# ziatdinovmax/GPim

Hardware: AMD Instinct MI355X
Metric: GP fit+predict grid-points/sec (higher is better)
Workload: dtype f64; 1 GPU; C2: 256x256 synthetic twisted-lattice image, 25% observed (N=16384, M=65536, d=2), Matern52 exact GP, T=100 Adam its (lr 0.1) + predict; one image per GPU; N=16384, M=65536, kernel=Matern52

## Files before the change

### gpim_amd/_lib.py

```python
import contextlib
import ctypes
import os

import torch

_HERE = os.path.dirname(os.path.abspath(__file__))
LIB_PATH = os.path.join(_HERE, "libgpimhip.so")

OK, E_BADARG, E_HIP, E_NOT_PD, E_NOMEM = 0, -1, -2, -3, -4
KERNEL_IDS = {"RBF": 0, "Matern52": 1, "RationalQuadratic": 2}
ACQ_IDS = {"cb": 0, "ei": 1, "poi": 2}
MAX_DIM, MAX_PARAMS = 4, 8

c_dp = ctypes.c_void_p


class ModelStruct(ctypes.Structure):
    _fields_ = [("kernel", ctypes.c_int32), ("dim", ctypes.c_int32), ("n_ls", ctypes.c_int32),
                ("reserved", ctypes.c_int32), ("amp_lo", ctypes.c_double), ("amp_hi", ctypes.c_double),
                ("ls_lo", ctypes.c_double * MAX_DIM), ("ls_hi", ctypes.c_double * MAX_DIM),
                ("jitter", ctypes.c_double)]


class VgpStruct(ctypes.Structure):
    _fields_ = [("tasks", ctypes.c_int32), ("rank", ctypes.c_int32), ("independent", ctypes.c_int32),
                ("ls_softplus", ctypes.c_int32)]


VGP_MAX_TASKS = 16


class SmStruct(ctypes.Structure):
    _fields_ = [("dim", ctypes.c_int32), ("mixtures", ctypes.c_int32), ("ard", ctypes.c_int32),
                ("reserved", ctypes.c_int32)]


SM_MAX_MIXTURES = 16


class GemmTestStruct(ctypes.Structure):
    _fields_ = [("A", c_dp), ("lda", ctypes.c_int64), ("a_roff", ctypes.c_int32), ("a_coff", ctypes.c_int32),
                ("B", c_dp), ("ldb", ctypes.c_int64), ("b_roff", ctypes.c_int32), ("b_coff", ctypes.c_int32),
                ("C", c_dp), ("ldc", ctypes.c_int64), ("c_roff", ctypes.c_int32), ("c_coff", ctypes.c_int32),
                ("colpart", c_dp), ("ld_colpart", ctypes.c_int64),
                ("alpha", ctypes.c_double), ("beta", ctypes.c_double),
                ("tiles", ctypes.POINTER(ctypes.c_int32)), ("ntiles", ctypes.c_int32),
                ("a_km", ctypes.c_int32), ("b_km", ctypes.c_int32), ("epi", ctypes.c_int32),
                ("krev", ctypes.c_int32), ("chunk", ctypes.c_int32), ("kfix0", ctypes.c_int32), ("kfix1", ctypes.c_int32),
                ("rect_rows", ctypes.c_int32), ("rect_cols", ctypes.c_int32), ("cj_max", ctypes.c_int32),
                ("cmap", ctypes.c_int32), ("rag", ctypes.c_int32), ("inplace", ctypes.c_int32),
                ("bshift", ctypes.c_int32), ("shape_div", ctypes.c_int32),
                ("sA", ctypes.c_int64), ("sB", ctypes.c_int64), ("sC", ctypes.c_int64), ("sColpart", ctypes.c_int64),
                ("batch", ctypes.c_int32)]


GEMM_SHAPES = {"quad": 0, "rowhalf": 1, "8w_lds": 2, "8w": 3, "4w": 4}
EPI_STORE, EPI_COLSUMSQ = 0, 1

_lib = None

_PROTOS = {
    "gpimhip_create": (ctypes.c_int, [ctypes.POINTER(ctypes.c_void_p), ctypes.c_int, ctypes.c_void_p]),
    "gpimhip_destroy": (ctypes.c_int, [ctypes.c_void_p]),
    "gpimhip_last_error": (ctypes.c_char_p, []),
    "gpimhip_version": (ctypes.c_int, []),
    "gpimhip_shutdown": (ctypes.c_int, []),
    "gpimhip_workspace_bytes": (ctypes.c_int64, [ctypes.c_void_p]),
    "gpimhip_sync": (ctypes.c_int, [ctypes.c_void_p]),
    "gpimhip_fit_completed": (ctypes.c_int, [ctypes.c_void_p]),
    "gpimhip_timing_enable": (ctypes.c_int, [ctypes.c_void_p, ctypes.c_int]),
    "gpimhip_timing_read": (ctypes.c_int, [ctypes.c_void_p, ctypes.c_int, ctypes.POINTER(ctypes.c_double),
                                           ctypes.POINTER(ctypes.c_int64)]),
    "gpimhip_kmat": (ctypes.c_int, [ctypes.c_void_p, ctypes.POINTER(ModelStruct), c_dp, ctypes.c_int64, c_dp,
                                    ctypes.c_int64, c_dp, ctypes.c_double, c_dp, ctypes.c_int64]),
    "gpimhip_potrf": (ctypes.c_int, [ctypes.c_void_p, c_dp, ctypes.c_int64, ctypes.c_int64, c_dp]),
    "gpimhip_nll_grad": (ctypes.c_int, [ctypes.c_void_p, ctypes.POINTER(ModelStruct), c_dp, c_dp, ctypes.c_int64,
                                        c_dp, c_dp, c_dp]),
    "gpimhip_fit_exact": (ctypes.c_int, [ctypes.c_void_p, ctypes.POINTER(ModelStruct), c_dp, c_dp, ctypes.c_int64,
                                         c_dp, ctypes.c_double, ctypes.c_int32, c_dp, c_dp]),
    "gpimhip_predict_exact": (ctypes.c_int, [ctypes.c_void_p, ctypes.POINTER(ModelStruct), c_dp, c_dp,
                                             ctypes.c_int64, c_dp, c_dp, ctypes.c_int64, c_dp, c_dp]),
    "gpimhip_sample_exact": (ctypes.c_int, [ctypes.c_void_p, ctypes.POINTER(ModelStruct), c_dp, c_dp, ctypes.c_int64,
                                            c_dp, c_dp, ctypes.c_int64, c_dp, ctypes.c_int32, ctypes.c_int32,
                                            ctypes.c_double, c_dp, c_dp, c_dp]),
    "gpimhip_sample_pathwise": (ctypes.c_int, [ctypes.c_void_p, ctypes.POINTER(ModelStruct), c_dp,
                                               ctypes.POINTER(ctypes.c_int32), ctypes.c_int32,
                                               ctypes.POINTER(ctypes.c_double), c_dp, c_dp, ctypes.c_int64, c_dp, c_dp,
                                               ctypes.c_int32, ctypes.c_int32, ctypes.c_double, c_dp, c_dp]),
    "gpimhip_sample_blocks": (ctypes.c_int, [ctypes.c_void_p, ctypes.POINTER(ModelStruct), c_dp,
                                             ctypes.POINTER(ctypes.c_int32), ctypes.c_int32,
                                             ctypes.POINTER(ctypes.c_double), c_dp, c_dp, c_dp,
                                             ctypes.c_int32, ctypes.c_int32, ctypes.c_double, c_dp, c_dp]),
    "gpimhip_sample_border": (ctypes.c_int, [ctypes.c_void_p, ctypes.POINTER(ModelStruct), c_dp, ctypes.c_int64, c_dp,
                                             ctypes.c_int64, ctypes.c_int32, c_dp, c_dp, ctypes.POINTER(ctypes.c_int32),
                                             ctypes.c_int32, ctypes.POINTER(ctypes.c_double), c_dp, c_dp, ctypes.c_int32,
                                             ctypes.c_int32, ctypes.c_double, c_dp, c_dp]),
    "gpimhip_fit_exact_batched": (ctypes.c_int, [ctypes.c_void_p, ctypes.POINTER(ModelStruct), c_dp, ctypes.c_int64,
                                                 c_dp, ctypes.c_int64, ctypes.c_int32, c_dp, ctypes.c_double,
                                                 ctypes.c_int32, c_dp, c_dp]),
    "gpimhip_predict_exact_batched": (ctypes.c_int, [ctypes.c_void_p, ctypes.POINTER(ModelStruct), c_dp,
                                                     ctypes.c_int64, c_dp, ctypes.c_int64, ctypes.c_int32, c_dp,
                                                     c_dp, ctypes.c_int64, c_dp, c_dp]),
    "gpimhip_vfe_nll_grad": (ctypes.c_int, [ctypes.c_void_p, ctypes.POINTER(ModelStruct), c_dp, c_dp, ctypes.c_int64,
                                            ctypes.c_int64, c_dp, c_dp, c_dp]),
    "gpimhip_fit_vfe": (ctypes.c_int, [ctypes.c_void_p, ctypes.POINTER(ModelStruct), c_dp, c_dp, ctypes.c_int64,
                                       ctypes.c_int64, c_dp, ctypes.c_double, ctypes.c_int32, c_dp, c_dp, c_dp]),
    "gpimhip_predict_vfe": (ctypes.c_int, [ctypes.c_void_p, ctypes.POINTER(ModelStruct), c_dp, c_dp, ctypes.c_int64,
                                           ctypes.c_int64, c_dp, c_dp, ctypes.c_int64, c_dp, c_dp]),
    "gpimhip_fit_vfe_batched": (ctypes.c_int, [ctypes.c_void_p, ctypes.POINTER(ModelStruct), c_dp, ctypes.c_int64, c_dp,
                                               ctypes.c_int64, ctypes.c_int64, ctypes.c_int32, c_dp, ctypes.c_double,
                                               ctypes.c_int32, c_dp, c_dp, c_dp]),
    "gpimhip_predict_vfe_batched": (ctypes.c_int, [ctypes.c_void_p, ctypes.POINTER(ModelStruct), c_dp, ctypes.c_int64, c_dp,
                                                   ctypes.c_int64, ctypes.c_int64, ctypes.c_int32, c_dp, c_dp,
                                                   ctypes.c_int64, ctypes.c_int64, c_dp, c_dp]),
    "gpimhip_kron_nll_grad": (ctypes.c_int, [ctypes.c_void_p, ctypes.POINTER(ModelStruct), ctypes.c_int32,
                                             ctypes.POINTER(ctypes.c_int32), c_dp, c_dp, c_dp, c_dp, c_dp]),
    "gpimhip_fit_kron": (ctypes.c_int, [ctypes.c_void_p, ctypes.POINTER(ModelStruct), ctypes.c_int32,
                                        ctypes.POINTER(ctypes.c_int32), c_dp, c_dp, c_dp, ctypes.c_double,
                                        ctypes.c_int32, c_dp, c_dp]),
    "gpimhip_predict_kron": (ctypes.c_int, [ctypes.c_void_p, ctypes.POINTER(ModelStruct), ctypes.c_int32,
                                            ctypes.POINTER(ctypes.c_int32), c_dp, c_dp, c_dp,
                                            ctypes.POINTER(ctypes.c_int32), c_dp, c_dp, c_dp]),
    "gpimhip_pkron_nll_grad": (ctypes.c_int, [ctypes.c_void_p, ctypes.POINTER(ModelStruct), c_dp, ctypes.c_int64, ctypes.c_int32,
                                              ctypes.c_int32, ctypes.POINTER(ctypes.c_int32), ctypes.POINTER(ctypes.c_int32),
                                              c_dp, c_dp, c_dp, c_dp, c_dp]),
    "gpimhip_fit_pkron": (ctypes.c_int, [ctypes.c_void_p, ctypes.POINTER(ModelStruct), c_dp, ctypes.c_int64, ctypes.c_int32,
                                         ctypes.c_int32, ctypes.POINTER(ctypes.c_int32), ctypes.POINTER(ctypes.c_int32),
                                         c_dp, c_dp, c_dp, ctypes.c_double, ctypes.c_int32, c_dp, c_dp]),
    "gpimhip_predict_pkron": (ctypes.c_int, [ctypes.c_void_p, ctypes.POINTER(ModelStruct), c_dp, ctypes.c_int64, ctypes.c_int32,
                                             ctypes.c_int32, ctypes.POINTER(ctypes.c_int32), ctypes.POINTER(ctypes.c_int32),
                                             c_dp, c_dp, c_dp, c_dp, ctypes.c_int64, ctypes.POINTER(ctypes.c_int32), c_dp,
                                             c_dp, c_dp]),
    "gpimhip_sample_pkron": (ctypes.c_int, [ctypes.c_void_p, ctypes.POINTER(ModelStruct), c_dp, ctypes.c_int64, ctypes.c_int32,
                                            ctypes.c_int32, ctypes.POINTER(ctypes.c_int32), ctypes.POINTER(ctypes.c_int32),
                                            c_dp, c_dp, c_dp, c_dp, ctypes.c_int64, ctypes.POINTER(ctypes.c_int32), c_dp,
                                            c_dp, ctypes.c_int64, ctypes.POINTER(ctypes.c_int32), ctypes.POINTER(ctypes.c_int32),
                                            ctypes.POINTER(ctypes.c_int32), c_dp, ctypes.POINTER(ctypes.c_int32),
                                            ctypes.POINTER(ctypes.c_int32), c_dp, ctypes.c_int32, ctypes.c_int32,
                                            ctypes.c_double, c_dp, c_dp]),
    "gpimhip_sample_kron": (ctypes.c_int, [ctypes.c_void_p, ctypes.POINTER(ModelStruct), ctypes.c_int32,
                                           ctypes.POINTER(ctypes.c_int32), c_dp, c_dp, c_dp,
                                           ctypes.POINTER(ctypes.c_int32), c_dp,
                                           ctypes.POINTER(ctypes.c_int32), c_dp,
                                           ctypes.POINTER(ctypes.c_int32), ctypes.POINTER(ctypes.c_int32),
                                           c_dp, ctypes.c_int32, ctypes.c_int32, ctypes.c_double, c_dp, c_dp]),
    "gpimhip_acq": (ctypes.c_int, [ctypes.c_void_p, ctypes.c_int32, c_dp, c_dp, ctypes.c_int64, ctypes.c_double,
                                   ctypes.c_double, c_dp, c_dp]),
    "gpimhip_nanmax": (ctypes.c_int, [ctypes.c_void_p, c_dp, ctypes.c_int64, c_dp]),
    "gpimhip_topk": (ctypes.c_int, [ctypes.c_void_p, c_dp, ctypes.c_int64, ctypes.c_int32, ctypes.c_int32,
                                    c_dp, c_dp, c_dp]),
    "gpimhip_dist_begin": (ctypes.c_int, [ctypes.c_void_p, ctypes.c_int64]),
    "gpimhip_dist_panel_factor": (ctypes.c_int, [ctypes.c_void_p, c_dp, ctypes.c_int64, ctypes.c_int32,
                                                 ctypes.c_int32, c_dp, c_dp]),
    "gpimhip_dist_setup": (ctypes.c_int, [ctypes.c_void_p, ctypes.c_int64, ctypes.c_int32, ctypes.c_int32]),
    "gpimhip_dist_panel_pack": (ctypes.c_int, [ctypes.c_void_p, c_dp, ctypes.c_int64, ctypes.c_int32, ctypes.c_int32,
                                               c_dp, ctypes.c_int64]),
    "gpimhip_dist_update": (ctypes.c_int, [ctypes.c_void_p, c_dp, ctypes.c_int64, ctypes.c_int32, c_dp, ctypes.c_int64,
                                           ctypes.c_int32, ctypes.c_int32]),
    "gpimhip_dist_solve_update": (ctypes.c_int, [ctypes.c_void_p, c_dp, ctypes.c_int64, ctypes.c_int32, c_dp,
                                                 ctypes.c_int64, ctypes.c_int64, c_dp, ctypes.c_int64, c_dp,
                                                 ctypes.c_int32]),
    "gpimhip_dist_solve_update2": (ctypes.c_int, [ctypes.c_void_p, c_dp, ctypes.c_int64, ctypes.c_int32, c_dp,
                                                  ctypes.c_int64, ctypes.c_int64, c_dp, ctypes.c_int64, c_dp,
                                                  ctypes.c_int32, ctypes.c_int32]),
    "gpimhip_dist_kmat_cols": (ctypes.c_int, [ctypes.c_void_p, ctypes.POINTER(ModelStruct), c_dp, ctypes.c_int64, c_dp,
                                              ctypes.c_int64, ctypes.c_int64, c_dp, ctypes.c_int64]),
    "gpimhip_dist_kinv_update": (ctypes.c_int, [ctypes.c_void_p, c_dp, ctypes.c_int64, ctypes.c_int32, c_dp,
                                                ctypes.c_int64, c_dp, ctypes.c_int64]),
    "gpimhip_dist_kinv_update_n": (ctypes.c_int, [ctypes.c_void_p, c_dp, ctypes.c_int64, ctypes.c_int32, ctypes.c_int32, c_dp,
                                                  ctypes.c_int64, c_dp, ctypes.c_int64]),
    "gpimhip_dist_grad_sums": (ctypes.c_int, [ctypes.c_void_p, ctypes.POINTER(ModelStruct), c_dp, ctypes.c_int64, c_dp,
                                              c_dp, ctypes.c_int64, c_dp, c_dp]),
    "gpimhip_dist_finalize": (ctypes.c_int, [ctypes.c_void_p, ctypes.POINTER(ModelStruct), ctypes.c_int64, c_dp, c_dp,
                                             ctypes.c_double, ctypes.c_double, ctypes.c_double, ctypes.c_int32, c_dp,
                                             c_dp, c_dp]),
    "gpimhip_dist_finalize_dev": (ctypes.c_int, [ctypes.c_void_p, ctypes.POINTER(ModelStruct), ctypes.c_int64, c_dp, c_dp,
                                                 c_dp, ctypes.c_double, ctypes.c_int32, c_dp, c_dp, c_dp]),
    "gpimhip_set_precision": (ctypes.c_int, [ctypes.c_void_p, ctypes.c_int32]),
    "gpimhip_set_reflection_shard": (ctypes.c_int, [ctypes.c_void_p, ctypes.c_int32, ctypes.c_int32, ctypes.c_int32, ctypes.c_int32]),
    "gpimhip_refl_sums": (ctypes.c_int, [ctypes.c_void_p, ctypes.POINTER(ModelStruct), c_dp, c_dp, ctypes.c_int64, ctypes.c_int32,
                                         c_dp, c_dp]),
    "gpimhip_set_reflection": (ctypes.c_int, [ctypes.c_void_p, ctypes.c_int32, ctypes.POINTER(ctypes.c_double), c_dp,
                                              ctypes.c_int64, ctypes.c_int64]),
    "gpimhip_set_border": (ctypes.c_int, [ctypes.c_void_p, ctypes.c_int32, ctypes.c_void_p, c_dp]),
    "gpimhip_nll_grad_batched": (ctypes.c_int, [ctypes.c_void_p, ctypes.POINTER(ModelStruct), c_dp, ctypes.c_int64, c_dp,
                                                ctypes.c_int64, ctypes.c_int32, c_dp, c_dp, c_dp]),
    "gpimhip_acquire_exact": (ctypes.c_int, [ctypes.c_void_p, ctypes.POINTER(ModelStruct), c_dp, c_dp, ctypes.c_int64,
                                             c_dp, c_dp, ctypes.c_int64, c_dp, ctypes.c_int64, ctypes.c_int32,
                                             ctypes.c_double, ctypes.c_double, c_dp, c_dp, c_dp, c_dp]),
    "gpimhip_thin_batch": (ctypes.c_int, [ctypes.c_void_p, c_dp, c_dp, ctypes.c_int32, ctypes.c_int32, c_dp,
                                          ctypes.c_double, ctypes.c_int32, c_dp, c_dp]),
    "gpimhip_dist_vec_forward": (ctypes.c_int, [ctypes.c_void_p, c_dp, ctypes.c_int64, ctypes.c_int32, ctypes.c_int32,
                                                c_dp, c_dp, c_dp, c_dp]),
    "gpimhip_dist_vec_backward": (ctypes.c_int, [ctypes.c_void_p, c_dp, ctypes.c_int64, ctypes.c_int32, ctypes.c_int32,
                                                 c_dp, c_dp, c_dp, c_dp]),
    "gpimhip_matvec_t": (ctypes.c_int, [ctypes.c_void_p, c_dp, ctypes.c_int64, ctypes.c_int64, ctypes.c_int64, c_dp,
                                        c_dp]),
    "gpimhip_step_plan_host": (ctypes.c_int, [ctypes.c_int32, ctypes.c_int32, ctypes.POINTER(ctypes.c_int32),
                                              ctypes.c_int64, ctypes.POINTER(ctypes.c_int64)]),
    "gpimhip_step_plan_host_f32": (ctypes.c_int, [ctypes.c_int32, ctypes.c_int32, ctypes.POINTER(ctypes.c_int32),
                                                  ctypes.c_int64, ctypes.POINTER(ctypes.c_int64),
                                                  ctypes.POINTER(ctypes.c_int32)]),
    "gpimhip_gemm_tiles": (ctypes.c_int, [ctypes.c_void_p, ctypes.POINTER(GemmTestStruct)]),
    "gpimhip_gemm_shape_host": (ctypes.c_int, [ctypes.c_int32, ctypes.c_int32, ctypes.c_int32, ctypes.c_int32,
                                               ctypes.c_int64, ctypes.c_int64, ctypes.c_int32, ctypes.c_int32]),
    "gpimhip_gemm_tile_pos_host": (ctypes.c_int, [ctypes.c_int32, ctypes.c_int32, ctypes.c_int32, ctypes.c_int32,
                                                  ctypes.c_int32, ctypes.c_int32, ctypes.POINTER(ctypes.c_int32),
                                                  ctypes.POINTER(ctypes.c_int32)]),
    "gpimhip_gemm_rect_tile_host": (ctypes.c_int, [ctypes.c_int32, ctypes.c_int32, ctypes.c_int32, ctypes.c_int32,
                                                   ctypes.POINTER(ctypes.c_int32), ctypes.POINTER(ctypes.c_int32)]),
    "gpimhip_kron_eigh": (ctypes.c_int, [ctypes.c_void_p, ctypes.c_int32, ctypes.POINTER(ctypes.c_int32), c_dp,
                                         ctypes.POINTER(ctypes.c_double), ctypes.c_int32, c_dp, c_dp,
                                         ctypes.POINTER(ctypes.c_int32), ctypes.POINTER(ctypes.c_int32),
                                         ctypes.POINTER(ctypes.c_double), ctypes.POINTER(ctypes.c_int32)]),
    "gpimhip_vgp_nll_grad": (ctypes.c_int, [ctypes.c_void_p, ctypes.POINTER(ModelStruct), ctypes.POINTER(VgpStruct), c_dp,
                                            c_dp, ctypes.c_int64, c_dp, c_dp, c_dp]),
    "gpimhip_fit_vgp": (ctypes.c_int, [ctypes.c_void_p, ctypes.POINTER(ModelStruct), ctypes.POINTER(VgpStruct), c_dp, c_dp,
                                       ctypes.c_int64, c_dp, ctypes.c_double, ctypes.c_int32, c_dp, c_dp]),
    "gpimhip_predict_vgp": (ctypes.c_int, [ctypes.c_void_p, ctypes.POINTER(ModelStruct), ctypes.POINTER(VgpStruct), c_dp,
                                           c_dp, ctypes.c_int64, c_dp, c_dp, ctypes.c_int64, c_dp, c_dp]),
    "gpimhip_sample_vgp": (ctypes.c_int, [ctypes.c_void_p, ctypes.POINTER(ModelStruct), ctypes.POINTER(VgpStruct), c_dp, c_dp,
                                          ctypes.c_int64, c_dp, c_dp, ctypes.c_int64, c_dp, ctypes.c_int32, ctypes.c_int32,
                                          ctypes.c_double, c_dp, c_dp, c_dp]),
    "gpimhip_sample_vgp_blocks": (ctypes.c_int, [ctypes.c_void_p, ctypes.POINTER(ModelStruct), ctypes.POINTER(VgpStruct), c_dp,
                                                 ctypes.POINTER(ctypes.c_int32), ctypes.c_int32,
                                                 ctypes.POINTER(ctypes.c_double), c_dp, c_dp, c_dp, ctypes.c_int32,
                                                 ctypes.c_int32, ctypes.c_double, c_dp, c_dp]),
    "gpimhip_sm_kmat": (ctypes.c_int, [ctypes.c_void_p, ctypes.POINTER(SmStruct), c_dp, ctypes.c_int64, c_dp, ctypes.c_int64,
                                       c_dp, c_dp, ctypes.c_int64]),
    "gpimhip_sm_nll_grad": (ctypes.c_int, [ctypes.c_void_p, ctypes.POINTER(SmStruct), c_dp, c_dp, ctypes.c_int64, c_dp, c_dp,
                                           c_dp]),
    "gpimhip_fit_sm": (ctypes.c_int, [ctypes.c_void_p, ctypes.POINTER(SmStruct), c_dp, c_dp, ctypes.c_int64, c_dp,
                                      ctypes.c_double, ctypes.c_int32, c_dp, c_dp]),
    "gpimhip_predict_sm": (ctypes.c_int, [ctypes.c_void_p, ctypes.POINTER(SmStruct), c_dp, c_dp, ctypes.c_int64, c_dp, c_dp,
                                          ctypes.c_int64, c_dp, c_dp]),
    "gpimhip_sample_sm": (ctypes.c_int, [ctypes.c_void_p, ctypes.POINTER(SmStruct), c_dp, c_dp, ctypes.c_int64, c_dp, c_dp,
                                         ctypes.c_int64, c_dp, ctypes.c_int32, ctypes.c_int32, ctypes.c_double, c_dp, c_dp,
                                         c_dp]),
    "gpimhip_sample_sm_pathwise": (ctypes.c_int, [ctypes.c_void_p, ctypes.POINTER(SmStruct), c_dp,
                                                  ctypes.POINTER(ctypes.c_int32), ctypes.c_int32,
                                                  ctypes.POINTER(ctypes.c_double), c_dp, c_dp, ctypes.c_int64, c_dp, c_dp,
                                                  ctypes.c_int32, ctypes.c_int32, ctypes.c_double, c_dp, c_dp]),
    "gpimhip_sample_sm_blocks": (ctypes.c_int, [ctypes.c_void_p, ctypes.POINTER(SmStruct), c_dp,
                                                ctypes.POINTER(ctypes.c_int32), ctypes.c_int32,
                                                ctypes.POINTER(ctypes.c_double), c_dp, c_dp, c_dp,
                                                ctypes.c_int32, ctypes.c_int32, ctypes.c_double, c_dp, c_dp]),
    "gpimhip_sm_nll_grad_batched": (ctypes.c_int, [ctypes.c_void_p, ctypes.POINTER(SmStruct), c_dp, c_dp, c_dp, ctypes.c_int64,
                                                   ctypes.c_int32, c_dp, c_dp, c_dp]),
    "gpimhip_fit_sm_batched": (ctypes.c_int, [ctypes.c_void_p, ctypes.POINTER(SmStruct), c_dp, c_dp, c_dp, ctypes.c_int64,
                                              ctypes.c_int32, c_dp, ctypes.c_double, ctypes.c_int32, c_dp, c_dp]),
    "gpimhip_predict_sm_batched": (ctypes.c_int, [ctypes.c_void_p, ctypes.POINTER(SmStruct), c_dp, c_dp, c_dp, ctypes.c_int64,
                                                  ctypes.c_int32, c_dp, c_dp, ctypes.c_int64, c_dp, c_dp]),
}
EXPORTS = tuple(_PROTOS)


def load():
    global _lib
    if _lib is not None:
        return _lib
    if not os.path.exists(LIB_PATH):
        raise RuntimeError(
            "gpim_amd: %s is missing -- build it with `python -m gpim_amd._build` "
            "(hipcc --offload-arch=gfx950). There is no CPU fallback." % LIB_PATH)
    try:
        lib = ctypes.CDLL(LIB_PATH)
    except OSError as e:
        raise RuntimeError("gpim_amd: cannot load %s: %s. There is no CPU fallback." % (LIB_PATH, e))
    for name, (res, args) in _PROTOS.items():
        fn = getattr(lib, name)
        fn.restype, fn.argtypes = res, args
    _lib = lib
    import atexit
    atexit.register(_shutdown)
    return lib


import weakref

_live = weakref.WeakSet()


def _shutdown():
    import gc
    gc.collect()
    for h in list(_live):
        try:
            h.close()
        except Exception:
            pass
    try:
        if torch.cuda.is_available() and torch.cuda.is_initialized():
            torch.cuda.synchronize()
            _lib.gpimhip_shutdown()
    except Exception:
        pass


def require_gpu():
    if not torch.cuda.is_available():
        raise RuntimeError("gpim_amd: no HIP device visible to torch; the MI355X engine has no CPU fallback")
    return torch.device("cuda", torch.cuda.current_device())


class NotPositiveDefiniteError(torch.linalg.LinAlgError if hasattr(torch.linalg, "LinAlgError") else RuntimeError):
    """Raised where torch.linalg.cholesky would raise in the reference (gpr.py:192,248)."""


def check(rc):
    if rc == OK:
        return
    msg = load().gpimhip_last_error().decode()
    if rc == E_NOT_PD:
        raise NotPositiveDefiniteError("linalg.cholesky: " + msg)
    if rc == E_BADARG:
        raise ValueError("gpimhip: bad argument. " + msg)
    if rc == E_NOMEM:
        raise MemoryError("gpimhip: " + msg)
    raise RuntimeError("gpimhip: HIP error. " + msg)


class Handle:

    def __init__(self, precision="double", stream=None):
        self.device = require_gpu()
        lib = load()
        h = ctypes.c_void_p()
        stream = (stream or torch.cuda.current_stream(self.device)).cuda_stream
        check(lib.gpimhip_create(ctypes.byref(h), self.device.index, ctypes.c_void_p(stream)))
        self._h = h
        self.lib = lib
        _live.add(self)
        self.precision = precision
        if precision == "single":
            check(lib.gpimhip_set_precision(h, 32))

    @property
    def h(self):
        return self._h

    def close(self):
        if getattr(self, "_h", None):
            self.lib.gpimhip_destroy(self._h)
            self._h = None

    def __del__(self):
        try:
            self.close()
        except Exception:
            pass


def ptr(t):
    if t is None:
        return None
    assert t.is_cuda and (t.is_contiguous() or (t.dim() == 2 and t.stride(1) == 1))
    return ctypes.c_void_p(t.data_ptr())


@contextlib.contextmanager
def reflection(handle, blocks, var_count=0, border=None, shard=None):
    lib, h = handle.lib, handle.h
    mode = lambda *args: check(lib.gpimhip_set_reflection(h, *args))
    mode(blocks.mask, blocks.twoc, ptr(blocks.wts), blocks.n_total, int(var_count))
    try:
        if border is not None:
            M, q_d, coef_d = border
            check(lib.gpimhip_set_border(h, M, None if q_d is None else ctypes.c_void_p(q_d.data_ptr()), ptr(coef_d)))
        if shard is not None:
            check(lib.gpimhip_set_reflection_shard(h, *(int(v) for v in shard)))
        yield
    finally:
        mode(0, None, None, 0, 0)
```

### gpim_amd/csrc/api.hip

```cpp
#include <math.h>
#include <stdio.h>
#include <string.h>
#include <stdlib.h>
#include <algorithm>
#include <chrono>
#include <atomic>
#include <mutex>
#include "common.hpp"
#include "border.hpp"
#include "vgp.hpp"
#include "pkron.hpp"
#include "sm.hpp"
#include "sample.hpp"

static thread_local std::string g_err;
void gpim_set_error(const std::string& s) { g_err = s; }

int deal_chunk(int ntiles) { return std::max(1, std::min(64, ntiles / 512)); }
#define EAGER_MIN_PANELS 12


static inline int64_t mat_doubles(const gpimhip_ctx* h, int64_t elements) { return h->fp32 ? (elements + 1) / 2 : elements; }

static void ws_release_matrix(gpimhip_ctx* h) {
    dev_release(h, h->A, h->B, h->Tm, h->dinv, h->dinvB, h->pcopy, h->ypad, h->z, h->alpha, h->logdet_part, h->grad_part,
                h->gemv_part, h->fin_counter, h->theta, h->adam_m, h->adam_v, h->iter);
    h->np = 0;
    h->ws_batch = 0;
}

int ws_ensure_b(gpimhip_ctx* h, int64_t N, int B, int padded, bool matrices) {
    const int64_t np = pad_to(std::max<int64_t>(N, 1), NB);
    const int64_t ld = np + ((padded && np >= 1024) ? (h->fp32 ? 32 : 16) : 0);
    if (np == h->np && B == h->ws_batch && ld == h->ld && (h->A != nullptr || !matrices)) return GPIMHIP_OK;
    HIP_TRY(hipStreamSynchronize(h->stream));
    ws_release_matrix(h);
    const int64_t nb = np / NB;
    h->np = np;
    h->ws_batch = B;
    h->ld = ld;
    int rc = GPIMHIP_OK;
    if ((matrices && ((rc = h->A.alloc(h, mat_doubles(h, B * np * ld))) ||
                      (rc = h->B.alloc(h, mat_doubles(h, B * np * ld))) ||
                      (rc = h->Tm.alloc(h, mat_doubles(h, B * np * ld))))) ||
        (rc = h->dinv.alloc(h, mat_doubles(h, B * nb * NB * NB))) ||
        (rc = h->dinvB.alloc(h, B * nb * NB * NB)) ||
        (rc = h->pcopy.alloc(h, (int64_t)B * NB * NB)) ||
        (rc = h->ypad.alloc(h, B * np)) || (rc = h->z.alloc(h, B * np)) ||
        (rc = h->alpha.alloc(h, B * np)) || (rc = h->logdet_part.alloc(h, B * nb)) ||
        (rc = h->grad_part.alloc(h, B * nb * (nb + 1) / 2 * 8)) || (rc = h->gemv_part.alloc(h, B * (int64_t)gemv_tri_chunks(np) * np)) || (rc = h->fin_counter.alloc(h, (int64_t)B)) || (rc = h->theta.alloc(h, (int64_t)B)) ||
        (rc = h->adam_m.alloc(h, (int64_t)B * MAXP)) || (rc = h->adam_v.alloc(h, (int64_t)B * MAXP)) ||
        (rc = h->iter.alloc(h, (int64_t)B))) {
        ws_release_matrix(h);
        return rc;
    }
    HIP_TRY(hipMemsetAsync(h->fin_counter, 0, (size_t)B * sizeof(uint32_t), h->stream));
    if (matrices) {
        HIP_TRY(hipMemsetAsync(h->Tm, 0, (size_t)mat_doubles(h, B * np * ld) * sizeof(double), h->stream));
        HIP_TRY(hipMemsetAsync(h->B, 0, (size_t)mat_doubles(h, B * np * ld) * sizeof(double), h->stream));
    }
    if (h->fp32 && h->refine.cap < 10 * (int64_t)B * np) {
        h->refine.release(h);
        if ((rc = h->refine.alloc(h, 10 * (int64_t)B * np))) {
            ws_release_matrix(h);
            return rc;
        }
    }
    if (matrices) {
        rc = plan_ensure(h, (int)nb);
        if (rc == GPIMHIP_OK) rc = h->fp32 ? step_plan_ensure(h, (int)nb) : step_plan_ensure_inv(h, (int)nb);
        if (rc != GPIMHIP_OK) { ws_release_matrix(h); return rc; }
    }
    return GPIMHIP_OK;
}
int ws_ensure(gpimhip_ctx* h, int64_t N) { return ws_ensure_b(h, N, h->nbatch, 0); }
static int ws_ensure_padded(gpimhip_ctx* h, int64_t N) { return ws_ensure_b(h, N, h->nbatch, 1); }

static void ws_release_predict(gpimhip_ctx* h) {
    dev_release(h, h->Ks, h->colpart, h->mean_tmp);
    for (auto& pl : h->pred_lists) pl.tiles.release(h);
    h->pred_lists.clear();
    h->pred_tiles = nullptr;
    h->pred_ntiles = 0;
    h->ks_rows = h->ks_cols = 0;
    h->ks_batch = 0;
}

int ws_ensure_predict(gpimhip_ctx* h, int64_t np, int64_t mc) {
    const int B = h->nbatch;
    if (!(h->ks_rows == np && h->ks_batch == B && mc <= h->ks_cols)) {
        HIP_TRY(hipStreamSynchronize(h->stream));
        const int64_t cap = (h->ks_rows == np && h->ks_batch == B) ? std::max(mc, h->ks_cols) : mc;
        ws_release_predict(h);
        h->ks_rows = np;
        h->ks_cols = cap;
        h->ks_batch = B;
        int rc = GPIMHIP_OK;
        if ((rc = h->Ks.alloc(h, mat_doubles(h, B * np * (cap + 16)))) || (rc = h->colpart.alloc(h, B * (np / NB) * cap)) ||
            (rc = h->mean_tmp.alloc(h, B * cap))) {
            ws_release_predict(h);
            return rc;
        }
    }
    const int nb = (int)(np / NB), nc = (int)(mc / NB);
    for (auto& pl : h->pred_lists)
        if (pl.nc == nc) {
            h->pred_tiles = pl.tiles;
            h->pred_ntiles = pl.tiles.cap;
            return GPIMHIP_OK;
        }
    std::vector<TileDesc> tl;
    tl.reserve((size_t)nb * nc);
    for (int ig = (nb - 1) / 8; ig >= 0; --ig)
        for (int jg = 0; jg <= (nc - 1) / 8; ++jg)
            for (int ci = std::min(nb - 1, ig * 8 + 7); ci >= ig * 8; --ci)
                for (int cj = jg * 8; cj < std::min(nc, jg * 8 + 8); ++cj) tl.push_back({ci, cj, 0, ci + 1});
    gpimhip_ctx::PredList pl{nc, {}};
    GP_TRY(pl.tiles.alloc(h, (int64_t)tl.size()));
    HIP_TRY(hipMemcpyAsync(pl.tiles, tl.data(), tl.size() * sizeof(TileDesc), hipMemcpyHostToDevice, h->stream));
    HIP_TRY(hipStreamSynchronize(h->stream));
    h->pred_lists.push_back(pl);
    h->pred_tiles = pl.tiles;
    h->pred_ntiles = pl.tiles.cap;
    return GPIMHIP_OK;
}

static void lower_patch_order(std::vector<TileDesc>& out, int lo, int hi, int kb0, int kb1) {
    for (int ig = lo / 8; ig <= (hi - 1) / 8; ++ig)
        for (int jg = lo / 8; jg <= ig; ++jg)
            for (int i = std::max(lo, ig * 8); i < std::min(hi, ig * 8 + 8); ++i)
                for (int j = std::max(lo, jg * 8); j < std::min(hi, jg * 8 + 8); ++j)
                    if (j <= i) out.push_back({i, j, kb0, kb1});
}

template <typename F>
static void rect_patch_order(std::vector<TileDesc>& out, int r0, int r1, int c0, int c1, bool rows_desc,
                             bool col_major, F krange) {
    const int nrg = (r1 - r0 + 7) / 8, ncg = (c1 - c0 + 7) / 8;
    const int nouter = col_major ? ncg : nrg, ninner = col_major ? nrg : ncg;
    for (int a = 0; a < nouter; ++a)
        for (int bq = 0; bq < ninner; ++bq) {
            int ig = col_major ? bq : a, jg = col_major ? a : bq;
            if (rows_desc) ig = nrg - 1 - ig;
            for (int i = r0 + ig * 8; i < std::min(r1, r0 + ig * 8 + 8); ++i)
                for (int j = c0 + jg * 8; j < std::min(c1, c0 + jg * 8 + 8); ++j) {
                    int k0, k1;
                    krange(i, j, k0, k1);
                    out.push_back({i, j, k0, k1});
                }
        }
}

struct TriNode { int lo, mid, hi; };
static int tri_build(int lo, int hi, std::vector<std::vector<TriNode>>& levels) {
    if (hi - lo <= 1) return 0;
    const int mid = lo + (hi - lo + 1) / 2;
    const int hl = tri_build(lo, mid, levels), hr = tri_build(mid, hi, levels);
    const int ht = 1 + std::max(hl, hr);
    if ((int)levels.size() < ht) levels.resize(ht);
    levels[ht - 1].push_back({lo, mid, hi});
    return ht;
}

int plan_ensure(gpimhip_ctx* h, int nb) {
    LinalgPlan& P = h->plan;
    if (P.nb == nb) return GPIMHIP_OK;
    if (P.d_tiles) { (void)hipFree(P.d_tiles); P.d_tiles = nullptr; }
    std::vector<TileDesc> tl;
    auto mark = [&](size_t start) { return PlanRange{(int64_t)start, (int32_t)(tl.size() - start)}; };
    std::vector<std::vector<TriNode>> levels;
    tri_build(0, nb, levels);
    P.tri_t.clear();
    P.tri_x.clear();
    auto sort_longest_first = [&](size_t nnodes, size_t start) {
        if (nnodes < 2 || tl.size() - start <= 512) return;
        std::stable_sort(tl.begin() + start, tl.end(),
                         [](const TileDesc& a, const TileDesc& b) { return a.kb1 - a.kb0 > b.kb1 - b.kb0; });
    };
    for (auto& lv : levels) {
        size_t s = tl.size();
        for (auto& nd : lv)
            rect_patch_order(tl, nd.mid, nd.hi, nd.lo, nd.mid, false, true,
                             [&](int, int cj, int& k0, int& k1) { k0 = cj; k1 = nd.mid; });
        sort_longest_first(lv.size(), s);
        P.tri_t.push_back(mark(s));
        s = tl.size();
        for (auto& nd : lv)
            rect_patch_order(tl, nd.mid, nd.hi, nd.lo, nd.mid, true, false,
                             [&](int ci, int, int& k0, int& k1) { k0 = nd.mid; k1 = ci + 1; });
        sort_longest_first(lv.size(), s);
        P.tri_x.push_back(mark(s));
    }
    {
        size_t s = tl.size();
        const int PR = 2, PC = 32;
        for (int ig = 0; ig <= (nb - 1) / PR; ++ig)
            for (int jg = 0; jg * PC <= std::min(nb - 1, ig * PR + PR - 1); ++jg)
                for (int i = ig * PR; i < std::min(nb, ig * PR + PR); ++i)
                    for (int j = jg * PC; j < std::min(nb, jg * PC + PC); ++j)
                        if (j <= i) tl.push_back({i, j, i, nb});
        P.lauum = mark(s);
    }
    P.n_tiles = (int64_t)tl.size();
    void* q = nullptr;
    HIP_TRY(hipMalloc(&q, std::max<size_t>(tl.size(), 1) * sizeof(TileDesc)));
    P.d_tiles = (TileDesc*)q;
    HIP_TRY(hipMemcpyAsync(P.d_tiles, tl.data(), tl.size() * sizeof(TileDesc), hipMemcpyHostToDevice, h->stream));
    HIP_TRY(hipStreamSynchronize(h->stream));
    P.nb = nb;
    return GPIMHIP_OK;
}

GemmArgs gemm_args(const double* A, int64_t lda, const double* B, int64_t ldb, double* C, int64_t ldc,
                   double alpha, double beta, const TileDesc* tiles, int n, int64_t rows) {
    GemmArgs g;
    memset(&g, 0, sizeof(g));
    g.A = A; g.lda = lda; g.B = B; g.ldb = ldb; g.C = C; g.ldc = ldc;
    g.alpha = alpha; g.beta = beta; g.tiles = tiles; g.ntiles = n;
    g.sA = rows * lda; g.sB = rows * ldb; g.sC = rows * ldc;
    return g;
}

struct SideStreams {
    hipStream_t capture = nullptr;
    bool capture_tried = false;
};
static std::mutex g_side_mutex;
static SideStreams g_side[64];
static std::atomic<int> g_side_generation{0};
static void side_refresh(gpimhip_ctx* h) {
    const int g = g_side_generation.load();
    if (h->side_generation == g) return;
    h->side_generation = g;
    h->capture_stream = nullptr;
    h->capture_stream_tried = false;
}
static std::mutex g_capture_mutex[64];
static void capture_lock(gpimhip_ctx* h) { g_capture_mutex[h->device & 63].lock(); }
static void capture_unlock(gpimhip_ctx* h) { g_capture_mutex[h->device & 63].unlock(); }

static hipStream_t ensure_capture_stream(gpimhip_ctx* h) {
    side_refresh(h);
    if (!h->capture_stream && !h->capture_stream_tried) {
        h->capture_stream_tried = true;
        std::lock_guard<std::mutex> lock(g_side_mutex);
        SideStreams& S = g_side[h->device & 63];
        if (!S.capture_tried) {
            S.capture_tried = true;
            if (hipStreamCreateWithFlags(&S.capture, hipStreamNonBlocking) != hipSuccess) S.capture = nullptr;
        }
        h->capture_stream = S.capture;
    }
    return h->capture_stream;
}

int launch_potrf(gpimhip_ctx* h, double* A, int64_t np, int64_t ld, int32_t* info) {
    return launch_potrf_steps(h, A, np, ld, info, nullptr);
}

int launch_trtri(gpimhip_ctx* h, double* A, double* Tm, int64_t np, int64_t ld) {
    const int nb = (int)(np / NB);
    GP_TRY(plan_ensure(h, nb));
    const LinalgPlan& P = h->plan;
    GP_TRY(launch_diag_inv_copy(h, A, ld, nb));
    for (size_t lv = 0; lv < P.tri_t.size(); ++lv) {
        GemmArgs g1 = gemm_args(A, ld, A, ld, Tm, ld, 1.0, 0.0, P.d_tiles + P.tri_t[lv].off, P.tri_t[lv].n, h->np);
        g1.chunk = deal_chunk(g1.ntiles);
        g1.krev = 1;
        GP_TRY(launch_gemm(h, false, true, EPI_STORE, g1));
        GemmArgs g2 = gemm_args(A, ld, Tm, ld, A, ld, -1.0, 0.0, P.d_tiles + P.tri_x[lv].off, P.tri_x[lv].n, h->np);
        g2.chunk = deal_chunk(g2.ntiles);
        GP_TRY(launch_gemm(h, false, true, EPI_STORE, g2));
    }
    return GPIMHIP_OK;
}

int launch_potrf_inv(gpimhip_ctx* h, double* A, double* Tm, int64_t np, int64_t ld, int32_t* info, int rag) {
    if (!h->fp32) return launch_potrf_steps(h, A, np, ld, info, Tm, rag);
    { StageTimer t(h, 0); GP_TRY(launch_potrf_steps(h, A, np, ld, info, nullptr)); }
    StageTimer t(h, 1);
    return launch_trtri(h, A, Tm, np, ld);
}

int launch_lauum(gpimhip_ctx* h, const double* A, double* B, int64_t np, int64_t ld, int rag) {
    const int nb = (int)(np / NB);
    GP_TRY(plan_ensure(h, nb));
    const LinalgPlan& P = h->plan;
    GemmArgs g = gemm_args(A, ld, A, ld, B, ld, 1.0, 0.0, P.d_tiles + P.lauum.off, P.lauum.n, h->np);
    g.chunk = deal_chunk(g.ntiles);
    g.krev = 1;
    g.rag = h->fp32 ? 0 : rag;
    return launch_gemm(h, true, true, EPI_STORE, g);
}

BorderWs* bws(const gpimhip_ctx* h) { return (BorderWs*)h->border; }
bool border_on(const gpimhip_ctx* h) { return h->refl.mask && h->border && bws(h)->M > 0; }

static void border_free_bufs(gpimhip_ctx* h, BorderWs* w) {
    dev_release(h, w->C, w->Y, w->tv, w->scal, w->uo, w->tiles_y, w->tiles_upd, w->R, w->rsq);
    w->np = 0; w->B = 0; w->n_y = w->n_upd = 0; w->r_cols = 0;
}
static void border_release(gpimhip_ctx* h) {
    BorderWs* w = bws(h);
    if (!w) return;
    border_free_bufs(h, w);
    if (w->sub) gpimhip_destroy(w->sub);
    delete w;
    h->border = nullptr;
}

static int border_ensure(gpimhip_ctx* h, int T = 1) {
    BorderWs* w = bws(h);
    const int64_t mp = pad_to(w->M, NB);
    if (!w->sub) GP_TRY(gpimhip_create(&w->sub, h->device, h->stream));
    w->sub->nbatch = T;
    w->sub->stream = h->stream;
    GP_TRY(ws_ensure_b(w->sub, w->M, T, 1));
    if (w->np == h->np && w->B == h->nbatch && w->T == T && w->mp == mp && w->C) return GPIMHIP_OK;
    HIP_TRY(hipStreamSynchronize(h->stream));
    border_free_bufs(h, w);
    w->mp = mp; w->np = h->np; w->B = h->nbatch; w->T = T;
    const int nb = (int)(h->np / NB), nm = (int)(mp / NB);
    std::vector<TileDesc> ty, tu;
    for (int ci = 0; ci < nb; ++ci)
        for (int cj = 0; cj < nm; ++cj) ty.push_back({ci, cj, 0, cj + 1});
    lower_patch_order(tu, 0, nb, 0, nm);
    w->n_y = (int)ty.size();
    w->n_upd = (int)tu.size();
    int rc = GPIMHIP_OK;
    if ((rc = w->C.alloc(h, (int64_t)w->B * w->np * mp)) || (rc = w->Y.alloc(h, (int64_t)w->B * w->np * mp)) ||
        (rc = w->tv.alloc(h, 2 * mp * T)) || (rc = w->scal.alloc(h, 2 * T)) || (rc = w->tiles_y.alloc(h, w->n_y)) ||
        (rc = w->tiles_upd.alloc(h, w->n_upd))) {
        border_free_bufs(h, w);
        return rc;
    }
    HIP_TRY(hipMemcpyAsync(w->tiles_y, ty.data(), ty.size() * sizeof(TileDesc), hipMemcpyHostToDevice, h->stream));
    HIP_TRY(hipMemcpyAsync(w->tiles_upd, tu.data(), tu.size() * sizeof(TileDesc), hipMemcpyHostToDevice, h->stream));
    HIP_TRY(hipStreamSynchronize(h->stream));
    return GPIMHIP_OK;
}
static int border_ensure_r(gpimhip_ctx* h, int64_t cols) {
    BorderWs* w = bws(h);
    if (w->r_cols >= cols && w->R) return GPIMHIP_OK;
    HIP_TRY(hipStreamSynchronize(h->stream));
    dev_release(h, w->R, w->rsq);
    w->r_cols = 0;
    int rc = GPIMHIP_OK;
    if ((rc = w->R.alloc(h, w->mp * cols * w->T)) || (rc = w->rsq.alloc(h, cols * w->T))) {
        w->R.release(h);
        return rc;
    }
    w->r_cols = cols;
    return GPIMHIP_OK;
}

static int border_iter(gpimhip_ctx* h, int64_t nq, bool update_inverse) {
    BorderWs* w = bws(h);
    gpimhip_ctx* sub = w->sub;
    sub->stream = h->stream;
    const int64_t mp = w->mp;
    GP_TRY(launch_border_gather_s(h, w, h->B, h->ld, sub->A, sub->ld));
    GP_TRY(launch_potrf_inv(sub, sub->A, sub->Tm, mp, sub->ld, sub->info, 0));
    GP_TRY(launch_border_tidy(h, w, sub->A, sub->ld));
    GP_TRY(launch_border_gather_c(h, w, h->B, h->ld, nq));
    {
        GemmArgs g = gemm_args(w->C, mp, sub->A, sub->ld, w->Y, mp, 1.0, 0.0, w->tiles_y, w->n_y, h->np);
        g.sB = sub->np * sub->ld;
        g.bshift = __builtin_ctz((unsigned)(h->nbatch / w->T));
        g.chunk = deal_chunk(g.ntiles);
        GP_TRY(launch_gemm(h, false, false, EPI_STORE, g));
    }
    GP_TRY(launch_border_vectors(h, w, sub->A, sub->ld, sub->logdet_part, (int)(mp / NB), h->alpha));
    if (update_inverse) {
// ... 1789 lines not shown
```

### gpim_amd/csrc/cholstep.hip

```cpp
#include <stdlib.h>
#include <string.h>
#include <algorithm>
#include <functional>
#include "potf2_body.hpp"
#include "gemm_body.hpp"

#ifndef STEP_W
#define STEP_W 4
#endif

#define TILE_COPY (1 << 19)

struct StepArgs {
    double* A; int64_t ld; int kblk; int nb;
    double* dinv_all; double* dinvB_all; double* logdet; int32_t* info;
    int col_off;
    int potf2;
    int pb_off, pb_cnt, hb_off, hb_cnt, swap;
    double* Tm;
    double* Pcopy;
    GemmArgs g;
};

template <int FTM, int FTN, bool ALONE, bool RAG = false>
__global__ __launch_bounds__(NTH, ALONE ? 2 : 4) void chol_step_kernel(StepArgs a) {
    constexpr int SM0 = POTF2_SMEM_DOUBLES > gemm_smem_doubles<FTM, FTN, 2>() ? POTF2_SMEM_DOUBLES : gemm_smem_doubles<FTM, FTN, 2>();
    static_assert(SM0 * 8 <= 80 * 1024, "two workgroups per CU");
    constexpr int SM = ALONE ? 84 * 128 : SM0;
    __shared__ __attribute__((aligned(16))) double smem[SM];
    const int b = a.swap ? blockIdx.y : blockIdx.x;
    const int by = a.swap ? blockIdx.x : blockIdx.y;
    if (b >= 8) {
        if (by >= a.hb_cnt) return;
        const int pb = by + a.hb_off;
        int quad;
        const int pos = gemm_tile_pos<FTM, FTN>(a.g.ntiles, a.g.chunk, b - 8, quad);
        TileDesc t = a.g.tiles[pos];
        const int kind = (t.kb1 >> 16) & 7;
        const bool copy = (t.kb1 & TILE_COPY) != 0;
        t.kb1 &= 0xffff;
        if (kind == 0) {
            if (copy && a.Pcopy) {
                GemmArgs g = a.g;
                g.C2 = a.Pcopy + (int64_t)pb * (NB * NB);
                gemm_tile_core<false, false, EPI_STORE, 8, FTM, FTN, 2, RAG>(g, t, quad, pb, smem);
            } else {
                gemm_tile_core<false, false, EPI_STORE, 8, FTM, FTN, 2, RAG>(a.g, t, quad, pb, smem);
            }
        } else {
            GemmArgs g = a.g;
            if (kind <= 2) { g.C = a.Tm; g.alpha = 1.0; g.beta = kind == 2 ? 1.0 : 0.0; }
            else { g.B = a.Tm; g.alpha = -1.0; g.beta = kind == 4 ? 1.0 : 0.0; }
            gemm_tile_core<false, true, EPI_STORE, 8, FTM, FTN, 2, RAG>(g, t, quad, pb, smem);
        }
        return;
    }
    if (b != 0 || !a.potf2 || by >= a.pb_cnt) return;
    if (!ALONE) __builtin_amdgcn_s_setprio(3);
    potf2_body<double, ALONE && FI_LOOKAHEAD>(smem, by + a.pb_off, a.A, a.ld, a.kblk, a.dinv_all, a.dinvB_all, a.logdet, a.info, a.nb,
                                              a.col_off, a.Tm != nullptr);
}

template <int WPE>
__global__ __launch_bounds__(256, WPE) void panel_solve_kernel(double* __restrict__ A, int64_t ld, int kblk, int nb,
                                                            const double* __restrict__ dinvB_all, int b_off) {
    constexpr int LDS_LD = 130;
    constexpr int ROWS = 32, MTS = ROWS / 16;
    __shared__ __attribute__((aligned(16))) double S[ROWS * LDS_LD];
    const int tid = threadIdx.x, lane = tid & 63, wave = tid >> 6;
    const int by = blockIdx.y + b_off;
    A += (int64_t)by * nb * NB * ld;
    const d2* DB = reinterpret_cast<const d2*>(dinvB_all + ((int64_t)by * nb + kblk) * (NB * NB));
    double* P = A + ((int64_t)(kblk + 1) * NB + (int64_t)blockIdx.x * ROWS) * ld + (int64_t)kblk * NB;
#pragma unroll
    for (int i = 0; i < ROWS / 4; ++i) {
        const int row = wave * (ROWS / 4) + i;
        __builtin_amdgcn_global_load_lds((const __attribute__((address_space(1))) void*)(P + (int64_t)row * ld + lane * 2),
                                         (__attribute__((address_space(3))) void*)(S + row * LDS_LD), 16, 0, 0);
    }
    const int t0 = wave, t1 = 7 - wave, n0 = 2 * t0 + 2;
    d2 bf[18];
#pragma unroll
    for (int q = 0; q < 18; ++q) {
        const int t = q < n0 ? t0 : t1, s2 = q < n0 ? q : q - n0;
        bf[q] = DB[(t * 16 + s2) * 64 + lane];
    }
    asm volatile("s_waitcnt vmcnt(0)" ::: "memory");
    __syncthreads();
    const d4 zero = (d4){0.0, 0.0, 0.0, 0.0};
    d4 acc[2][MTS];
#pragma unroll
    for (int x = 0; x < 2; ++x)
#pragma unroll
        for (int mt = 0; mt < MTS; ++mt) acc[x][mt] = zero;
    const double* Sa = S + (lane & 15) * LDS_LD + (lane >> 4);
#pragma unroll
    for (int q = 0; q < 18; ++q) {
        const bool first = q < n0;
        const int s2 = first ? q : q - n0;
#pragma unroll
        for (int e = 0; e < 2; ++e) {
            const int s = 2 * s2 + e;
#pragma unroll
            for (int mt = 0; mt < MTS; ++mt) {
                const double av = Sa[mt * 16 * LDS_LD + 4 * s];
                if (first) acc[0][mt] = __builtin_amdgcn_mfma_f64_16x16x4f64(av, bf[q][e], acc[0][mt], 0, 0, 0);
                else acc[1][mt] = __builtin_amdgcn_mfma_f64_16x16x4f64(av, bf[q][e], acc[1][mt], 0, 0, 0);
            }
        }
    }
#pragma unroll
    for (int x = 0; x < 2; ++x) {
        const int t = x == 0 ? t0 : t1;
#pragma unroll
        for (int mt = 0; mt < MTS; ++mt)
#pragma unroll
            for (int rg = 0; rg < 4; ++rg)
                P[(int64_t)(mt * 16 + (lane >> 4) + 4 * rg) * ld + t * 16 + (lane & 15)] = acc[x][mt][rg];
    }
}

__global__ __launch_bounds__(256, 2) void diag_update_kernel(double* __restrict__ A, int64_t ld, int kblk, int nb, int b_off) {
    constexpr int LDS_LD = 130;
    __shared__ __attribute__((aligned(16))) double S[64 * LDS_LD];
    const int tid = threadIdx.x, lane = tid & 63, wave = tid >> 6;
    A += (int64_t)(blockIdx.y + b_off) * nb * NB * ld;
    const int jj = kblk + 1 + blockIdx.x / 10, q = blockIdx.x % 10;
    const int a = q < 1 ? 0 : q < 3 ? 1 : q < 6 ? 2 : 3, b = q - a * (a + 1) / 2;
    const double* Pa = A + ((int64_t)jj * NB + a * 32) * ld + (int64_t)kblk * NB;
    const double* Pb = A + ((int64_t)jj * NB + b * 32) * ld + (int64_t)kblk * NB;
#pragma unroll
    for (int i = 0; i < 8; ++i) {
        const int row = wave * 8 + i;
        __builtin_amdgcn_global_load_lds((const __attribute__((address_space(1))) void*)(Pa + (int64_t)row * ld + lane * 2),
                                         (__attribute__((address_space(3))) void*)(S + row * LDS_LD), 16, 0, 0);
        __builtin_amdgcn_global_load_lds((const __attribute__((address_space(1))) void*)(Pb + (int64_t)row * ld + lane * 2),
                                         (__attribute__((address_space(3))) void*)(S + (32 + row) * LDS_LD), 16, 0, 0);
    }
    const int wm = wave >> 1, wn = wave & 1;
    double* C = A + ((int64_t)jj * NB + a * 32 + wm * 16 + (lane >> 4)) * ld + (int64_t)jj * NB + b * 32 + wn * 16 + (lane & 15);
    double cv[4];
#pragma unroll
    for (int rg = 0; rg < 4; ++rg) cv[rg] = C[(int64_t)(4 * rg) * ld];
    asm volatile("s_waitcnt vmcnt(0)" ::: "memory");
    __syncthreads();
    d4 acc0 = (d4){0.0, 0.0, 0.0, 0.0}, acc1 = acc0;
    const double* Sa = S + (wm * 16 + (lane & 15)) * LDS_LD + (lane >> 4);
    const double* Sb = S + (32 + wn * 16 + (lane & 15)) * LDS_LD + (lane >> 4);
#pragma unroll
    for (int s = 0; s < 32; s += 2) {
        acc0 = __builtin_amdgcn_mfma_f64_16x16x4f64(Sa[4 * s], Sb[4 * s], acc0, 0, 0, 0);
        acc1 = __builtin_amdgcn_mfma_f64_16x16x4f64(Sa[4 * s + 4], Sb[4 * s + 4], acc1, 0, 0, 0);
    }
#pragma unroll
    for (int rg = 0; rg < 4; ++rg) C[(int64_t)(4 * rg) * ld] = cv[rg] - (acc0[rg] + acc1[rg]);
}

template <int ROWS>
__global__ __launch_bounds__(512, 2) void panel_solve_diag_kernel(double* __restrict__ A, int64_t ld, int kblk, int nb,
                                                                  const double* __restrict__ dinvB_all,
                                                                  const double* __restrict__ Pcopy, int b_off) {
    constexpr int LDS_LD = 130, MTS = ROWS / 16, NS = NB / ROWS, NDIAG = NS * (NS + 1) / 2;
    __shared__ __attribute__((aligned(16))) double S[2 * ROWS * LDS_LD];
    const int tid = threadIdx.x, lane = tid & 63, wave = (tid >> 6) & 3, half = tid >> 8;
    const int by = blockIdx.y + b_off;
    A += (int64_t)by * nb * NB * ld;
    Pcopy += (int64_t)by * (NB * NB);
    const d2* DB = reinterpret_cast<const d2*>(dinvB_all + ((int64_t)by * nb + kblk) * (NB * NB));
    const bool diag = blockIdx.x < NDIAG;
    int a = 0, b = 0;
    if (diag) {
        const int q = blockIdx.x;
        while ((a + 1) * (a + 2) / 2 <= q) ++a;
        b = q - a * (a + 1) / 2;
    }
    const int jj = kblk + 1;
    const int strip = diag ? (half == 0 ? a : b) : NS + 2 * (int)(blockIdx.x - NDIAG) + half;
    const bool work = !diag || half == 0 || b != a;
    double* P = A + ((int64_t)jj * NB + strip * ROWS) * ld + (int64_t)kblk * NB;
    double* Ss = S + half * ROWS * LDS_LD;
    if (work) {
#pragma unroll
        for (int i = 0; i < ROWS / 4; ++i) {
            const int row = wave * (ROWS / 4) + i;
            const double* src = diag ? Pcopy + (strip * ROWS + row) * NB + lane * 2 : P + (int64_t)row * ld + lane * 2;
            __builtin_amdgcn_global_load_lds((const __attribute__((address_space(1))) void*)src,
                                             (__attribute__((address_space(3))) void*)(Ss + row * LDS_LD), 16, 0, 0);
        }
    }
    const int t0 = wave, t1 = 7 - wave, n0 = 2 * t0 + 2;
    d2 bf[18];
    if (work) {
#pragma unroll
        for (int q = 0; q < 18; ++q) {
            const int t = q < n0 ? t0 : t1, s2 = q < n0 ? q : q - n0;
            bf[q] = DB[(t * 16 + s2) * 64 + lane];
        }
    }
    const int wt = tid >> 6, wm = wt / MTS, wn = wt % MTS;
    const bool syrk = diag && wt < MTS * MTS;
    double* C = A + ((int64_t)jj * NB + a * ROWS + wm * 16 + (lane >> 4)) * ld + (int64_t)jj * NB + b * ROWS + wn * 16 + (lane & 15);
    double cv[4] = {0.0, 0.0, 0.0, 0.0};
    if (syrk) {
#pragma unroll
        for (int rg = 0; rg < 4; ++rg) cv[rg] = C[(int64_t)(4 * rg) * ld];
    }
    asm volatile("s_waitcnt vmcnt(0)" ::: "memory");
    __syncthreads();
    const d4 zero = (d4){0.0, 0.0, 0.0, 0.0};
    d4 acc[2][MTS];
#pragma unroll
    for (int x = 0; x < 2; ++x)
#pragma unroll
        for (int mt = 0; mt < MTS; ++mt) acc[x][mt] = zero;
    if (work) {
        const double* Sa = Ss + (lane & 15) * LDS_LD + (lane >> 4);
#pragma unroll
        for (int q = 0; q < 18; ++q) {
            const bool first = q < n0;
            const int s2 = first ? q : q - n0;
#pragma unroll
            for (int e = 0; e < 2; ++e) {
                const int s = 2 * s2 + e;
#pragma unroll
                for (int mt = 0; mt < MTS; ++mt) {
                    const double av = Sa[mt * 16 * LDS_LD + 4 * s];
                    if (first) acc[0][mt] = __builtin_amdgcn_mfma_f64_16x16x4f64(av, bf[q][e], acc[0][mt], 0, 0, 0);
                    else acc[1][mt] = __builtin_amdgcn_mfma_f64_16x16x4f64(av, bf[q][e], acc[1][mt], 0, 0, 0);
                }
            }
        }
        if (!diag || (a == b && half == 0)) {
#pragma unroll
            for (int x = 0; x < 2; ++x) {
                const int t = x == 0 ? t0 : t1;
#pragma unroll
                for (int mt = 0; mt < MTS; ++mt)
#pragma unroll
                    for (int rg = 0; rg < 4; ++rg)
                        P[(int64_t)(mt * 16 + (lane >> 4) + 4 * rg) * ld + t * 16 + (lane & 15)] = acc[x][mt][rg];
            }
        }
    }
    if (!diag) return;
    __syncthreads();
    if (work) {
#pragma unroll
        for (int x = 0; x < 2; ++x) {
            const int t = x == 0 ? t0 : t1;
#pragma unroll
            for (int mt = 0; mt < MTS; ++mt)
#pragma unroll
                for (int rg = 0; rg < 4; ++rg)
                    Ss[(mt * 16 + (lane >> 4) + 4 * rg) * LDS_LD + t * 16 + (lane & 15)] = acc[x][mt][rg];
        }
    }
    __syncthreads();
    if (!syrk) return;
    d4 acc0 = zero, acc1 = zero;
    const double* Sa = S + (wm * 16 + (lane & 15)) * LDS_LD + (lane >> 4);
    const double* Sb = S + ((b != a ? ROWS : 0) + wn * 16 + (lane & 15)) * LDS_LD + (lane >> 4);
#pragma unroll
    for (int s = 0; s < 32; s += 2) {
        acc0 = __builtin_amdgcn_mfma_f64_16x16x4f64(Sa[4 * s], Sb[4 * s], acc0, 0, 0, 0);
        acc1 = __builtin_amdgcn_mfma_f64_16x16x4f64(Sa[4 * s + 4], Sb[4 * s + 4], acc1, 0, 0, 0);
    }
#pragma unroll
    for (int rg = 0; rg < 4; ++rg) C[(int64_t)(4 * rg) * ld] = cv[rg] - (acc0[rg] + acc1[rg]);
}

static void lower_patches(std::vector<TileDesc>& out, int lo, int hi, int kb0, int kb1) {
    for (int ig = lo / 8; ig <= (hi - 1) / 8; ++ig)
        for (int jg = lo / 8; jg <= ig; ++jg)
            for (int i = std::max(lo, ig * 8); i < std::min(hi, ig * 8 + 8); ++i)
                for (int j = std::max(lo, jg * 8); j < std::min(hi, jg * 8 + 8); ++j)
                    if (j <= i) out.push_back({i, j, kb0, kb1});
}

static bool pair_mode32(int nb) { return nb >= 160; }
static int fill_cap32(int nb) { return pair_mode32(nb) ? 64 : (nb < 88 ? (1 << 30) : 128); }

struct HostSim {
    std::vector<double> slot;
    double makespan = 0.0;
    explicit HostSim(int S) : slot(S, 0.0) {}
    static double cost(const TileDesc& t) { return ((t.kb1 & 0xffff) - t.kb0) + 0.5; }
    double peek() const { return slot.front(); }
    void add(double c) {
        std::pop_heap(slot.begin(), slot.end(), std::greater<double>());
        slot.back() += c;
        makespan = std::max(makespan, slot.back());
        std::push_heap(slot.begin(), slot.end(), std::greater<double>());
    }
    bool try_add(double c, int q, double limit) {
        double t[4];
        for (int w = 0; w < q; ++w) {
            std::pop_heap(slot.begin(), slot.end() - w, std::greater<double>());
            t[w] = slot[slot.size() - 1 - w];
        }
        const bool ok = t[q - 1] + c <= limit;
        for (int w = q - 1; w >= 0; --w) {
            if (ok) { slot[slot.size() - 1 - w] = t[w] + c; makespan = std::max(makespan, t[w] + c); }
            std::push_heap(slot.begin(), slot.end() - w, std::greater<double>());
        }
        return ok;
    }
};
#define HOST_SLOTS 512
static double wg_cost(int depth, int q) { return q == 4 ? 0.14 * depth + 0.24 : (q == 2 ? 0.34 * depth + 0.3 : depth + 0.5); }

static void plan_updates(int nb, std::vector<std::vector<TileDesc>>& fill) {
#ifndef STEP_W_CHAIN
#define STEP_W_CHAIN 3
#endif
#ifndef STEP_W_CHAIN_MIN
#define STEP_W_CHAIN_MIN 16
#endif
    const int W = (nb >= STEP_W_CHAIN_MIN && nb < 64) ? STEP_W_CHAIN : STEP_W, S = HOST_SLOTS;
    const int npanel = (nb + W - 1) / W;
    auto by_depth = [](const TileDesc& a, const TileDesc& b) { return (a.kb1 - a.kb0) > (b.kb1 - b.kb0); };
    auto col_update = [&](std::vector<TileDesc>& tl, int p0, int j) {
        const int kb0 = std::max(0, p0 - W);
        if (j > kb0)
            for (int i = j + 1; i < nb; ++i) tl.push_back({i, j, kb0, j});
        if (j + 1 < nb) {
            const int kd = std::max(0, ((j + 1) / W) * W - W);
            if (j > kd) tl.push_back({j + 1, j + 1, kd, j});
        }
    };
    if (nb < 64) {
        for (int p = 0; p < npanel; ++p) {
            const int p0 = p * W, p1 = std::min(p0 + W, nb), ncol = p1 - p0;
            std::vector<TileDesc> bulk;
            if (p > 0 && p0 + W < nb) lower_patches(bulk, p0 + W, nb, p0 - W, p0);
            const size_t per = (bulk.size() + ncol - 1) / ncol;
            size_t taken = 0;
            for (int j = p0; j < p1; ++j) {
                col_update(fill[j], p0, j);
                for (size_t q = 0; q < per && taken < bulk.size(); ++q) fill[j].push_back(bulk[taken++]);
            }
        }
        return;
    }
    std::vector<int> pend((size_t)nb * nb, 0);
    for (int p = 0; p < npanel; ++p) {
        const int p0 = p * W, p1 = std::min(p0 + W, nb);
        const int rem = nb - p0 - W;
        std::vector<TileDesc> req, opt;
        if (p > 0 && rem > 0) {
            const int c0 = p0 + W, c1 = std::min(p0 + 2 * W, nb);
            for (int i = c0; i < nb; ++i)
                for (int jj = c0; jj < std::min(c1, i + 1); ++jj) req.push_back({i, jj, pend[(size_t)i * nb + jj], p0});
            if (c1 < nb) lower_patches(opt, c1, nb, 0, p0);
            for (auto& t : opt) t.kb0 = pend[(size_t)t.ci * nb + t.cj];
        }
        const bool bulk_regime = rem >= 64;
#ifndef PLAN_FLUSH
#define PLAN_FLUSH 2
#endif
        constexpr int F = PLAN_FLUSH;
        auto due = [&](const TileDesc& t) { return (t.kb1 - t.kb0) >= F * W || (((t.ci >> 3) + (t.cj >> 3)) % F) == (p % F); };
        double due_cost = 0.0;
        size_t n_due = 0;
        if (bulk_regime) {
            std::stable_sort(opt.begin(), opt.end(), [&](const TileDesc& a, const TileDesc& b) {
                const int da = due(a), db = due(b);
                if (da != db) return da > db;
                return da ? by_depth(a, b) : false;
            });
            for (auto& t : opt)
                if (due(t)) { ++n_due; due_cost += HostSim::cost(t); }
        }
        size_t rtaken = 0, otaken = 0;
        for (int j = p0; j < p1; ++j) {
            const int left = p1 - j;
            std::vector<TileDesc>& tl = fill[j];
            col_update(tl, p0, j);
            const size_t nreq = (req.size() - rtaken + left - 1) / left;
            for (size_t q = 0; q < nreq; ++q) tl.push_back(req[rtaken++]);
            if (!bulk_regime) {
                const size_t nopt = (opt.size() - otaken + left - 1) / left;
                for (size_t q = 0; q < nopt; ++q) tl.push_back(opt[otaken++]);
            } else {
                HostSim sim(S);
                sim.add(1.0);
                std::stable_sort(tl.begin(), tl.end(), by_depth);
                double base = 0.0;
                for (auto& t : tl) { sim.add(HostSim::cost(t)); base += HostSim::cost(t); }
                const double per_slot = (base + due_cost / left) / S;
                const double unit = F * W + 0.5;
                const double target = std::max(sim.makespan, unit * std::max(1.0, std::floor(per_slot / unit + 0.5)));
                double got = 0.0;
                while (otaken < opt.size() && sim.peek() + HostSim::cost(opt[otaken]) <= target + 0.25) {
                    const double c = HostSim::cost(opt[otaken]);
                    sim.add(c);
                    if (otaken < n_due) got += c;
                    tl.push_back(opt[otaken++]);
                }
                due_cost -= std::min(due_cost, got);
            }
            std::stable_sort(tl.begin(), tl.end(), by_depth);
            for (auto& t : tl)
                if (t.cj >= p0 + W) pend[(size_t)t.ci * nb + t.cj] = t.kb1;
        }
    }
}

enum { TK_UPDATE = 0, TK_T_FIRST = 1, TK_T_ACC = 2, TK_X_FIRST = 3, TK_X_ACC = 4 };
struct TriOp { int ci, cj, k0, k1, kp; };
struct TriNodeS {
    int lo, mid, hi, left, right, height;
    int t_done = 1 << 30, x_done = 1 << 30;
    std::vector<TriOp> T, X;
    size_t t_open = 0, x_open = 0;
};
static int tri_nodes(int lo, int hi, std::vector<TriNodeS>& nodes) {
    TriNodeS n;
    n.lo = lo; n.hi = hi; n.mid = lo; n.left = n.right = -1; n.height = 0;
    if (hi - lo <= 1) {
        n.t_done = n.x_done = lo;
        nodes.push_back(n);
        return (int)nodes.size() - 1;
    }
    n.mid = lo + (hi - lo + 1) / 2;
    n.left = tri_nodes(lo, n.mid, nodes);
    n.right = tri_nodes(n.mid, hi, nodes);
    n.height = 1 + std::max(nodes[n.left].height, nodes[n.right].height);
    for (int cj = lo; cj < n.mid; ++cj)
        for (int ci = n.mid; ci < hi; ++ci) n.T.push_back({ci, cj, cj, n.mid, cj});
    for (int ci = hi - 1; ci >= n.mid; --ci)
        for (int cj = lo; cj < n.mid; ++cj) n.X.push_back({ci, cj, n.mid, ci + 1, n.mid});
    n.t_open = n.T.size();
    n.x_open = n.X.size();
    nodes.push_back(n);
    return (int)nodes.size() - 1;
}

#ifndef BATCH_QUAD_MAX
#define BATCH_QUAD_MAX 700
#endif
static int host_shape(int64_t update_kblocks, int quad_max = 2000) { return update_kblocks <= quad_max ? 4 : (update_kblocks <= 2800 ? 2 : 1); }

#ifndef PAIR_MIN_QUADS
#define PAIR_MIN_QUADS 300
#endif
#ifndef PAIR_MIN_DEPTH10
#define PAIR_MIN_DEPTH10 30
#endif
static bool pair_rule(size_t ntiles, int64_t kblocks) { return 4 * ntiles >= PAIR_MIN_QUADS && 10 * kblocks >= PAIR_MIN_DEPTH10 * (int64_t)ntiles; }
static bool plan_inverse(int nb, std::vector<std::vector<TileDesc>>& fill, std::vector<std::vector<TileDesc>>& post,
                         std::vector<uint8_t>& pair) {
    std::vector<TriNodeS> nodes;
    tri_nodes(0, nb, nodes);
    std::vector<int> order(nodes.size());
    for (size_t i = 0; i < order.size(); ++i) order[i] = (int)i;
    std::stable_sort(order.begin(), order.end(), [&](int a, int b) { return nodes[a].height < nodes[b].height; });
    size_t open_nodes = 0;
    for (auto& n : nodes) open_nodes += (n.height > 0);
#ifndef PLAN_CHAIN
#define PLAN_CHAIN 0.8
#endif
    const double CHAIN = PLAN_CHAIN;
    for (int L = 0; open_nodes > 0; ++L) {
        const bool hosted = L < nb;
        if (!hosted) post.emplace_back();
        std::vector<TileDesc>& out = hosted ? fill[L] : post.back();
        int64_t upd = 0;
        for (auto& t : out) upd += t.kb1 - t.kb0;
        const int q = hosted ? host_shape(upd) : 1;
        const int cd = !hosted ? (1 << 20) : 6;
        const bool two = hosted && q == 4 && pair_rule(out.size(), upd);
        if (hosted) pair[L] = two;
#ifndef PLAN_PAIR_SLOW
#define PLAN_PAIR_SLOW 1.7
#endif
#ifndef PLAN_PAIR_CHAIN
#define PLAN_PAIR_CHAIN 0.3
#endif
        const double slow = two ? PLAN_PAIR_SLOW : 1.0, chain = two ? CHAIN + PLAN_PAIR_CHAIN : CHAIN;
        HostSim sim(q == 1 || two ? HOST_SLOTS : HOST_SLOTS / 2);
        double target = 1e30;
        if (hosted) {
            sim.add(chain);
            for (auto& t : out)
                for (int w = 0; w < q; ++w) sim.add(slow * wg_cost(t.kb1 - t.kb0, q));
            target = std::max(sim.makespan, chain);
        }
        bool full = false;
        for (int idx : order) {
            TriNodeS& n = nodes[idx];
            if (n.height == 0 || n.x_open == 0 || full) continue;
            const bool t_phase = n.t_open > 0;
            if (t_phase ? !(nodes[n.left].x_done < L && n.mid <= L) : !(n.t_done < L && nodes[n.right].x_done < L && n.hi <= L)) continue;
            std::vector<TriOp>& ops = t_phase ? n.T : n.X;
            size_t& open = t_phase ? n.t_open : n.x_open;
            for (auto& o : ops) {
                if (o.kp >= o.k1) continue;
                int depth = std::min(o.k1 - o.kp, cd);
                if (hosted) {
                    while (depth >= 1 && !sim.try_add(slow * wg_cost(depth, q), q, target + 0.02)) --depth;
                    if (depth < 1) { full = true; break; }
                } else {
                    for (int w = 0; w < q; ++w) sim.add(wg_cost(depth, q));
                }
                const int k1 = o.kp + depth;
                const int kind = t_phase ? (o.kp == o.k0 ? TK_T_FIRST : TK_T_ACC) : (o.kp == o.k0 ? TK_X_FIRST : TK_X_ACC);
                out.push_back({o.ci, o.cj, o.kp, k1 | (kind << 16)});
                o.kp = k1;
                if (o.kp >= o.k1 && --open == 0) {
                    if (t_phase) n.t_done = L;
                    else { n.x_done = L; --open_nodes; }
                }
            }
        }
        std::stable_sort(out.begin(), out.end(), [](const TileDesc& a, const TileDesc& b) {
            return ((a.kb1 & 0xffff) - a.kb0) > ((b.kb1 & 0xffff) - b.kb0);
        });
        if (!hosted && out.empty()) post.pop_back();
        if (L > nb + 4 * 64) return false;
    }
    return true;
}

static void plan_updates_f32(int nb, std::vector<std::vector<TileDesc>>& fill, std::vector<std::vector<TileDesc>>& rest,
                             std::vector<int>& ndiag) {
    const int W = STEP_W;
    const int npanel = (nb + W - 1) / W;
    fill.assign(nb, {});
    rest.assign(npanel, {});
    ndiag.assign(nb, 0);
    for (int p = 0; p < npanel; ++p) {
        const int p0 = p * W, p1 = std::min(p0 + W, nb), ncol = p1 - p0;
        std::vector<TileDesc> bulk;
        if (p > 0 && p0 + W < nb) {
            if (!pair_mode32(nb)) {
                lower_patches(bulk, p0 + W, nb, p0 - W, p0);
            } else if ((p - 1) % 2 == 0) {
                const int c0 = p0 + W, c1 = std::min(p0 + 2 * W, nb);
                for (int ig = c0 / 8; ig <= (nb - 1) / 8; ++ig)
                    for (int i = std::max(c0, ig * 8); i < std::min(nb, ig * 8 + 8); ++i)
                        for (int j = c0; j < std::min(c1, i + 1); ++j) bulk.push_back({i, j, p0 - W, p0});
            } else {
                lower_patches(bulk, p0 + W, nb, p0 - 2 * W, p0);
            }
        }
        const size_t per = std::min<size_t>((size_t)fill_cap32(nb), (bulk.size() + ncol - 1) / ncol);
        size_t taken = 0;
        for (int j = p0; j < p1; ++j) {
            const int kb0 = std::max(0, p0 - W);
            if (j > kb0)
                for (int i = j + 1; i < nb; ++i) fill[j].push_back({i, j, kb0, j});
            for (size_t q = 0; q < per && taken < bulk.size(); ++q) fill[j].push_back(bulk[taken++]);
        }
        while (taken < bulk.size()) rest[p].push_back(bulk[taken++]);
    }
    for (int j = 0; j < nb; ++j) {
        const int p1 = std::min((j / W) * W + W, nb);
        ndiag[j] = std::max(0, std::min(nb, p1 + W) - (j + 1));
    }
}

static int step_plan_build(gpimhip_ctx* h, int nb, StepPlan& P, bool with_inverse) {
    const bool fp32 = h->fp32 != 0;
    if (P.nb == nb && P.fp32 == (int)fp32) return GPIMHIP_OK;
    if (P.d_tiles) { (void)hipFree(P.d_tiles); P.d_tiles = nullptr; }
    const int W = STEP_W;
    const int npanel = (nb + W - 1) / W;
    std::vector<std::vector<TileDesc>> fill(nb), post, rest(npanel);
    std::vector<int> ndiag32;
    if (!fp32) plan_updates(nb, fill);
    else plan_updates_f32(nb, fill, rest, ndiag32);
    P.n_update.assign(nb, 0);
    for (int j = 0; j < nb; ++j)
        for (auto& t : fill[j]) P.n_update[j] += t.kb1 - t.kb0;
    P.pair.assign(nb, 0);
    if (with_inverse) {
        if (!plan_inverse(nb, fill, post, P.pair)) {
            gpim_set_error("step plan: the inverse's tile operations did not all find a launch (nb = " + std::to_string(nb) + ")");
            return GPIMHIP_E_BADARG;
        }
    } else {
        for (int j = 0; j < nb; ++j) P.pair[j] = host_shape(P.n_update[j]) == 4 && pair_rule(fill[j].size(), P.n_update[j]);
    }
    P.n_all.assign(nb, 0);
    for (int j = 0; j < nb; ++j)
        for (auto& t : fill[j]) P.n_all[j] += (t.kb1 & 0xffff) - t.kb0;
    std::vector<TileDesc> tl;
    auto put = [&](const std::vector<TileDesc>& v) {
        PlanRange r{(int64_t)tl.size(), (int32_t)v.size()};
        tl.insert(tl.end(), v.begin(), v.end());
        return r;
    };
    P.fill.assign(nb, {0, 0});
    P.diag.assign(nb, {0, 0});
    P.bulk_rest.assign(npanel, {0, 0});
    P.post.clear();
    P.copy.assign(nb, 0);
    for (int j = 0; j < nb; ++j) {
        if (!fp32)
            for (TileDesc& t : fill[j])
                if ((t.kb1 >> 16) == TK_UPDATE && t.ci == j + 1 && t.cj == j) { t.kb1 |= TILE_COPY; P.copy[j] = 1; }
        P.fill[j] = put(fill[j]);
        P.diag[j] = PlanRange{0, fp32 ? ndiag32[j] : (j + 1 < nb ? 1 : 0)};
    }
    for (int p = 0; p < npanel; ++p) P.bulk_rest[p] = put(rest[p]);
    for (auto& v : post) P.post.push_back(put(v));
    P.n_tiles = (int64_t)tl.size();
    void* q = nullptr;
    HIP_TRY(hipMalloc(&q, std::max<size_t>(tl.size(), 1) * sizeof(TileDesc)));
    P.d_tiles = (TileDesc*)q;
    HIP_TRY(hipMemcpyAsync(P.d_tiles, tl.data(), tl.size() * sizeof(TileDesc), hipMemcpyHostToDevice, h->stream));
    HIP_TRY(hipStreamSynchronize(h->stream));
    P.nb = nb;
    P.fp32 = (int)fp32;
    return GPIMHIP_OK;
}

static int64_t emit_plan_records(int launch, const std::vector<TileDesc>& v, int32_t* out, int64_t cap, int64_t n) {
    for (const TileDesc& t : v) {
        if (out && n < cap) {
            int32_t* r = out + 6 * n;
            r[0] = launch; r[1] = t.ci; r[2] = t.cj; r[3] = t.kb0; r[4] = t.kb1 & 0xffff; r[5] = t.kb1 >> 16;
        }
        ++n;
    }
    return n;
}

extern "C" int gpimhip_step_plan_host(int32_t nb, int32_t with_inverse, int32_t* out, int64_t cap, int64_t* n_out) {
    if (nb < 1 || nb > 4096 || !n_out) return GPIMHIP_E_BADARG;
    std::vector<std::vector<TileDesc>> fill(nb), post;
    plan_updates(nb, fill);
    std::vector<uint8_t> pair(nb, 0);
    if (with_inverse && !plan_inverse(nb, fill, post, pair)) return GPIMHIP_E_BADARG;
    int64_t n = 0;
    for (int j = 0; j < nb; ++j) n = emit_plan_records(j, fill[j], out, cap, n);
    for (size_t q = 0; q < post.size(); ++q) n = emit_plan_records(nb + (int)q, post[q], out, cap, n);
    *n_out = n;
    return GPIMHIP_OK;
}

extern "C" int gpimhip_step_plan_host_f32(int32_t nb, int32_t with_inverse, int32_t* out, int64_t cap, int64_t* n_out,
                                          int32_t* diag_out) {
    if (nb < 1 || nb > 4096 || !n_out) return GPIMHIP_E_BADARG;
    std::vector<std::vector<TileDesc>> fill, rest, post;
    std::vector<int> ndiag;
    plan_updates_f32(nb, fill, rest, ndiag);
    std::vector<uint8_t> pair(nb, 0);
    if (with_inverse && !plan_inverse(nb, fill, post, pair)) return GPIMHIP_E_BADARG;
    int64_t n = 0;
    for (int j = 0; j < nb; ++j) n = emit_plan_records(j, fill[j], out, cap, n);
    for (size_t p = 0; p < rest.size(); ++p) n = emit_plan_records(-((int)p + 1), rest[p], out, cap, n);
    for (size_t q = 0; q < post.size(); ++q) n = emit_plan_records(nb + (int)q, post[q], out, cap, n);
    if (diag_out)
        for (int j = 0; j < nb; ++j) diag_out[j] = ndiag[j];
    *n_out = n;
    return GPIMHIP_OK;
}

int step_plan_ensure(gpimhip_ctx* h, int nb) { return step_plan_build(h, nb, h->splan, false); }
int step_plan_ensure_inv(gpimhip_ctx* h, int nb) { return step_plan_build(h, nb, h->splan_inv, true); }

void step_plan_release(gpimhip_ctx* h) {
    for (StepPlan* P : {&h->splan, &h->splan_inv}) {
        if (P->d_tiles) (void)hipFree(P->d_tiles);
        P->d_tiles = nullptr;
        P->nb = 0;
    }
}

static GemmArgs nt_update(double* A, int64_t ld, const TileDesc* tiles, int n, int64_t rows) {
    GemmArgs g;
    memset(&g, 0, sizeof(g));
    g.A = A; g.lda = ld; g.B = A; g.ldb = ld; g.C = A; g.ldc = ld;
    g.alpha = -1.0; g.beta = 1.0; g.tiles = tiles; g.ntiles = n;
    g.sA = g.sB = g.sC = rows * ld;
    return g;
}

static int launch_step(gpimhip_ctx* h, StepArgs& a, bool potf2, int n, int q, const int* split = nullptr, bool two_per_cu = false) {
    const int B = h->nbatch;
    a.potf2 = potf2 ? 1 : 0;
    if (!potf2 && n == 0) return GPIMHIP_OK;
    a.pb_off = a.hb_off = 0; a.pb_cnt = a.hb_cnt = B; a.swap = 0;
    dim3 grid(n ? 8 + q * n : 1, B);
    bool alone = potf2;
    if (q == 4 && two_per_cu) alone = false;
    if (split) {
        a.pb_off = split[0]; a.pb_cnt = potf2 ? split[1] : 0; a.hb_off = split[2]; a.hb_cnt = n ? split[3] : 0; a.swap = 1;
        grid = dim3(std::max(a.pb_cnt, a.hb_cnt), n ? 8 + q * n : 1);
        alone = false;
        if (grid.x == 0) return GPIMHIP_OK;
        if (grid.y > 65535) { gpim_set_error("step launch: tile list too long for a split batch"); return GPIMHIP_E_BADARG; }
    }
    if (a.g.rag && n) {
        if (q == 4 && alone) hipLaunchKernelGGL((chol_step_kernel<64, 64, true, true>), grid, dim3(NTH), 0, h->stream, a);
        else if (q == 4) hipLaunchKernelGGL((chol_step_kernel<64, 64, false, true>), grid, dim3(NTH), 0, h->stream, a);
        else if (q == 2) hipLaunchKernelGGL((chol_step_kernel<128, 64, false, true>), grid, dim3(NTH), 0, h->stream, a);
        else hipLaunchKernelGGL((chol_step_kernel<128, 128, false, true>), grid, dim3(NTH), 0, h->stream, a);
    } else if (q == 4 && alone) hipLaunchKernelGGL((chol_step_kernel<64, 64, true>), grid, dim3(NTH), 0, h->stream, a);
    else if (q == 4) hipLaunchKernelGGL((chol_step_kernel<64, 64, false>), grid, dim3(NTH), 0, h->stream, a);
    else if (q == 2) hipLaunchKernelGGL((chol_step_kernel<128, 64, false>), grid, dim3(NTH), 0, h->stream, a);
    else hipLaunchKernelGGL((chol_step_kernel<128, 128, false>), grid, dim3(NTH), 0, h->stream, a);
    HIP_TRY(hipGetLastError());
    return GPIMHIP_OK;
}

static int launch_solve_diag(gpimhip_ctx* h, double* A, int64_t ld, int j, int nb, int ndiag, int b_off, int cnt,
                             bool fused = false) {
    if (j + 1 >= nb || cnt <= 0) return GPIMHIP_OK;
    if (fused && cnt <= 4) {
        const int below = nb - j - 2;
        if ((36 + 4 * below) * cnt <= 256)
            hipLaunchKernelGGL(panel_solve_diag_kernel<16>, dim3(36 + 4 * below, cnt), dim3(512), 0, h->stream, A, ld, j, nb,
                               (const double*)h->dinvB, (const double*)h->pcopy, b_off);
        else
            hipLaunchKernelGGL(panel_solve_diag_kernel<32>, dim3(10 + 2 * below, cnt), dim3(512), 0, h->stream, A, ld, j, nb,
                               (const double*)h->dinvB, (const double*)h->pcopy, b_off);
        HIP_TRY(hipGetLastError());
        return GPIMHIP_OK;
    }
    if (cnt > 4)
        hipLaunchKernelGGL(panel_solve_kernel<4>, dim3(4 * (nb - j - 1), cnt), dim3(256), 0, h->stream, A, ld, j, nb,
                           (const double*)h->dinvB, b_off);
    else
        hipLaunchKernelGGL(panel_solve_kernel<2>, dim3(4 * (nb - j - 1), cnt), dim3(256), 0, h->stream, A, ld, j, nb,
                           (const double*)h->dinvB, b_off);
    HIP_TRY(hipGetLastError());
    if (ndiag > 0) {
        hipLaunchKernelGGL(diag_update_kernel, dim3(10 * ndiag, cnt), dim3(256), 0, h->stream, A, ld, j, nb, b_off);
        HIP_TRY(hipGetLastError());
    }
    return GPIMHIP_OK;
}

int launch_potrf_steps(gpimhip_ctx* h, double* A, int64_t np, int64_t ld, int32_t* info, double* Tm, int rag) {
    if (h->fp32) return launch_potrf_steps_f32(h, A, np, ld, info);
    const int nb = (int)(np / NB);
    if (Tm) GP_TRY(step_plan_ensure_inv(h, nb));
    else GP_TRY(step_plan_ensure(h, nb));
    const StepPlan& P = Tm ? h->splan_inv : h->splan;
    const int B = h->nbatch;
    const int host_max_batch = 4;
    StepArgs a;
    a.A = A; a.ld = ld; a.nb = nb; a.Tm = Tm;
    a.dinv_all = h->dinv; a.dinvB_all = h->dinvB; a.logdet = h->logdet_part; a.info = info;
    a.col_off = 0;
    a.Pcopy = h->pcopy;
    const bool no_fused = getenv("GPIMHIP_NO_FUSED_FD") != nullptr;
    auto fused = [&](int j) { return !no_fused && h->pcopy && P.copy[j] && P.diag[j].n == 1 && !(rag && j + 2 == nb); };
    {
        StageTimer t(h, 0);
        auto hosted_list = [&](int j, int problems, int& q) {
            const int nf = P.fill[j].n;
            a.g = nt_update(A, ld, P.d_tiles + P.fill[j].off, nf, h->np);
            a.g.chunk = std::max(1, std::min(64, nf / 512));
            a.g.rag = rag;
            q = B > host_max_batch ? host_shape((int64_t)P.n_all[j] * problems, BATCH_QUAD_MAX) : host_shape((int64_t)P.n_update[j] * problems);
            return nf;
        };
        if (B > host_max_batch) {
            const int c0 = (B + 1) / 2, c1 = B - c0;
            int q;
            int nf = hosted_list(0, c0, q);
            const int first[4] = {0, 0, 0, c0};
            GP_TRY(launch_step(h, a, false, nf, q, first));
            for (int j = 0; j < nb; ++j) {
                a.kblk = j;
                nf = hosted_list(j, c1, q);
                const int sa[4] = {0, c0, c0, c1};
                GP_TRY(launch_step(h, a, true, nf, q, sa));
                GP_TRY(launch_solve_diag(h, A, ld, j, nb, P.diag[j].n, 0, c0, fused(j)));
                nf = j + 1 < nb ? hosted_list(j + 1, c0, q) : 0;
                const int sb[4] = {c0, c1, 0, c0};
                GP_TRY(launch_step(h, a, true, nf, q, sb));
                GP_TRY(launch_solve_diag(h, A, ld, j, nb, P.diag[j].n, c0, c1, fused(j)));
            }
        } else {
            for (int j = 0; j < nb; ++j) {
                a.kblk = j;
                int q;
                const int nf = hosted_list(j, B, q);
                GP_TRY(launch_step(h, a, true, nf, q, nullptr, P.pair[j] != 0));
                GP_TRY(launch_solve_diag(h, A, ld, j, nb, P.diag[j].n, 0, B, fused(j)));
            }
        }
    }
    if (Tm) {
        StageTimer t(h, 1);
        a.kblk = -1;
        for (const PlanRange& r : P.post) {
            a.g = nt_update(A, ld, P.d_tiles + r.off, r.n, h->np);
            a.g.chunk = std::max(1, std::min(64, r.n / 512));
            a.g.rag = rag;
            const int64_t nt = (int64_t)r.n * B;
            GP_TRY(launch_step(h, a, false, r.n, nt <= 320 ? 4 : (nt <= 1000 ? 2 : 1)));
        }
    }
    return GPIMHIP_OK;
}

int launch_panel_chain(gpimhip_ctx* h, double* A, int64_t ld, int p0, int p1, int nb, const TileDesc* tiles,
                       const PlanRange* colfill, int32_t* info) {
    const int B = h->nbatch;
    StepArgs a;
    a.A = A; a.ld = ld; a.nb = nb; a.Tm = nullptr;
    a.dinv_all = h->dinv; a.dinvB_all = h->dinvB; a.logdet = h->logdet_part; a.info = info;
    a.col_off = 0;
    a.Pcopy = nullptr;
    for (int j = p0; j < p1; ++j) {
        a.kblk = j;
        const PlanRange f = colfill[j - p0];
        a.g = nt_update(A, ld, tiles + f.off, f.n, h->np);
        a.g.chunk = 1;
        GP_TRY(launch_step(h, a, true, f.n, f.n <= 128 ? 4 : 2));
        GP_TRY(launch_solve_diag(h, A, ld, j, nb, std::max(0, p1 - j - 1), 0, B));
    }
    return GPIMHIP_OK;
}
```

### gpim_amd/csrc/common.hpp

```cpp
#pragma once
#include <hip/hip_runtime.h>
#include <stdint.h>
#include <functional>
#include <string>
#include <vector>
#include <utility>
#include "../../include/gpimhip.h"

#define NB 128
#define GEMM_BK 16
#define MAXP GPIMHIP_MAX_PARAMS

void gpim_set_error(const std::string& s);

#define HIP_TRY(expr)                                                              \
    do {                                                                           \
        hipError_t _e = (expr);                                                    \
        if (_e != hipSuccess) {                                                    \
            gpim_set_error(std::string(#expr) + ": " + hipGetErrorString(_e));     \
            return GPIMHIP_E_HIP;                                                  \
        }                                                                          \
    } while (0)

#define GP_TRY(expr)                      \
    do {                                  \
        int _r = (expr);                  \
        if (_r != GPIMHIP_OK) return _r;  \
    } while (0)

struct gpimhip_ctx;
template <typename T> struct DevBuf {
    T* p = nullptr;
    int64_t cap = 0;
    int alloc(gpimhip_ctx* h, int64_t count, const char* what = nullptr);
    int grow(gpimhip_ctx* h, int64_t want);
    void release(gpimhip_ctx* h);
    operator T*() const { return p; }
};

struct TileDesc {
    int32_t ci, cj, kb0, kb1;
};

struct ThetaDev {
    double var;
    double ls[GPIMHIP_MAX_DIM];
    double inv_ls[GPIMHIP_MAX_DIM];
    double noise;
    double alpha;
    double diag_add;
    double dvar_du;
    double dls_du[GPIMHIP_MAX_DIM];
    double dnoise_du;
    double dalpha_du;
};

struct AdamStep {
    double lr_over_bc1;
    double bc2_sqrt;
    double beta1, beta2, eps;
};
static inline AdamStep adam_step_init() {
    AdamStep st;
    st.beta1 = 0.9; st.beta2 = 0.999; st.eps = 1e-8; st.lr_over_bc1 = 0.0; st.bc2_sqrt = 1.0;
    return st;
}

struct FinalizeIter {
    int32_t* iter;
    const double* bc;
    int32_t T;
    double* hist_base;
    double* loss_base;
};

struct PlanRange { int64_t off; int32_t n; };

struct LinalgPlan {
    int nb = 0;
    TileDesc* d_tiles = nullptr;
    int64_t n_tiles = 0;
    std::vector<PlanRange> tri_t, tri_x;
    PlanRange lauum{0, 0};
};

struct StepPlan {
    int nb = 0;
    int fp32 = 0;
    TileDesc* d_tiles = nullptr;
    int64_t n_tiles = 0;
    std::vector<PlanRange> fill;
    std::vector<PlanRange> diag;
    std::vector<PlanRange> bulk_rest;
    std::vector<PlanRange> post;
    std::vector<int32_t> n_update;
    std::vector<int32_t> n_all;
    std::vector<uint8_t> pair;
    std::vector<uint8_t> copy;
};

struct DistPlan {
    int nb = 0, world = 0, rank = 0;
    TileDesc* d_tiles = nullptr;
    int64_t n_tiles = 0;
    std::vector<PlanRange> colfill;
    std::vector<PlanRange> upd_panel;
    std::vector<PlanRange> kinv_panel;
    PlanRange grad_tiles{0, 0};
    int rect_cols = 0;
    TileDesc* d_rect = nullptr;
    int64_t n_rect = 0;
};

struct ReflArgs {
    int mask;
    double twoc[GPIMHIP_MAX_DIM];
    const double* wts;
    int64_t n_total;
    int64_t var_count;
    int pb_off, pb_stride, nblocks_total, raw;
};
struct gpimhip_ctx {
    ReflArgs refl = {0, {0, 0, 0, 0}, nullptr, 0, 0, 0, 1, 0, 0};
    int device = 0;
    hipStream_t stream = nullptr;
    hipStream_t capture_stream = nullptr;
    bool capture_stream_tried = false;
    int side_generation = 0;
    int64_t np = 0;
    int64_t ld = 0;
    int nbatch = 1;
    int ws_batch = 0;
    DevBuf<double> A;
    DevBuf<double> B;
    DevBuf<double> Tm;
    DevBuf<double> dinv;
    DevBuf<double> dinvB;
    DevBuf<double> pcopy;
    DevBuf<double> ypad;
    DevBuf<double> z;
    DevBuf<double> alpha;
    DevBuf<double> logdet_part;
    DevBuf<double> grad_part;
    DevBuf<double> gemv_part;
    DevBuf<uint32_t> fin_counter;
    DevBuf<ThetaDev> theta;
    DevBuf<ThetaDev> theta1;
    DevBuf<int32_t> iter;
    DevBuf<double> adam_m;
    DevBuf<double> adam_v;
    DevBuf<int32_t> info;
    int64_t ks_rows = 0, ks_cols = 0, ks_batch = 0;
    struct PredList { int nc; DevBuf<TileDesc> tiles; };
    std::vector<PredList> pred_lists;
    DevBuf<double> Ks;
    DevBuf<double> colpart;
    DevBuf<double> mean_tmp;
    TileDesc* pred_tiles = nullptr;
    int64_t pred_ntiles = 0;
    int64_t bytes = 0;
    LinalgPlan plan;
    StepPlan splan, splan_inv;
    DistPlan dplan;
    bool timing = false;
    std::vector<std::pair<hipEvent_t, hipEvent_t>> ev[7];
    DevBuf<double> bc;
    std::vector<double> bc_host;
    DevBuf<unsigned long long> keys;
    DevBuf<double> acq_tmp;
    DevBuf<char> sel_scratch;
    int fit_completed = 0;
    int32_t* pinned_info = nullptr;
    hipEvent_t ra_ev[2] = {nullptr, nullptr};
    void* vfe = nullptr;
    void* kron = nullptr;
    void* vgp = nullptr;
    void* pkron = nullptr;
    void* sm = nullptr;
    void* border = nullptr;
    void* sample = nullptr;
    DevBuf<double> refine;
    int fp32 = 0;
};

template <typename T> int DevBuf<T>::alloc(gpimhip_ctx* h, int64_t count, const char* what) {
    void* q = nullptr;
    hipError_t e = hipMalloc(&q, (size_t)count * sizeof(T));
    if (e != hipSuccess) {
        if (what) (void)hipGetLastError();
        gpim_set_error(what ? std::string(what) : std::string("hipMalloc failed: ") + hipGetErrorString(e));
        return GPIMHIP_E_NOMEM;
    }
    p = (T*)q;
    cap = count;
    h->bytes += cap * (int64_t)sizeof(T);
    return GPIMHIP_OK;
}
template <typename T> void DevBuf<T>::release(gpimhip_ctx* h) {
    if (p) {
        (void)hipFree(p);
        h->bytes -= cap * (int64_t)sizeof(T);
    }
    p = nullptr;
    cap = 0;
}
template <typename T> int DevBuf<T>::grow(gpimhip_ctx* h, int64_t want) {
    if (cap >= want) return GPIMHIP_OK;
    HIP_TRY(hipStreamSynchronize(h->stream));
    release(h);
    return alloc(h, want);
}
template <typename... Bufs> static inline void dev_release(gpimhip_ctx* h, Bufs&... bufs) { (bufs.release(h), ...); }

struct BatchScope {
    gpimhip_ctx* h; int prev;
    BatchScope(gpimhip_ctx* h_, int nbatch) : h(h_), prev(h_->nbatch) { h->nbatch = nbatch; }
    ~BatchScope() { h->nbatch = prev; }
};

#define FP64_ONLY(h)                                                                                      \
    do {                                                                                                  \
        if ((h) && (h)->fp32) {                                                                           \
            gpim_set_error("this entry point needs a double-precision handle (gpimhip_set_precision(h, 64))"); \
            return GPIMHIP_E_BADARG;                                                                      \
        }                                                                                                 \
    } while (0)

static inline int64_t pad_to(int64_t n, int64_t m) { return (n + m - 1) / m * m; }
struct Carve {
    double* base;
    int64_t used = 0;
    explicit Carve(double* b) : base(b) {}
    template <typename T = double> T* take(int64_t doubles) {
        const int64_t off = (used + 1) & ~(int64_t)1;
        used = off + doubles;
        return base ? (T*)(base + off) : nullptr;
    }
};
static inline int rag_of(int64_t N, int64_t np) {
    const int64_t last = N - (np - NB);
    return (np >= 2 * NB && last > 0 && last <= 64) ? (int)(np / NB) : 0;
}

struct StageTimer {
    gpimhip_ctx* h; int stage; hipEvent_t e1 = nullptr;
    StageTimer(gpimhip_ctx* h_, int s) : h(h_), stage(s) {
        if (!h->timing) return;
        hipEvent_t e0;
        if (hipEventCreate(&e0) != hipSuccess || hipEventCreate(&e1) != hipSuccess) { e1 = nullptr; return; }
        (void)hipEventRecord(e0, h->stream);
        h->ev[stage].push_back({e0, e1});
    }
    ~StageTimer() { if (e1) (void)hipEventRecord(e1, h->stream); }
};

static inline int gemv_tri_rc(int64_t np) {
    const int64_t rc = ((np / 32 + NB - 1) / NB) * NB;
    return (int)(rc < NB ? NB : (rc > 1024 ? 1024 : rc));
}
static inline int gemv_tri_chunks(int64_t np) { return (int)((np + gemv_tri_rc(np) - 1) / gemv_tri_rc(np)); }
#define OUTER_W 4
int ws_ensure(gpimhip_ctx* h, int64_t N);
int ws_ensure_b(gpimhip_ctx* h, int64_t N, int B, int padded, bool matrices = true);
int ws_ensure_predict(gpimhip_ctx* h, int64_t np, int64_t mc);
int deal_chunk(int ntiles = 1 << 30);
int model_state_at_u(gpimhip_ctx* h, const gpimhip_model_t* m, const double* X, int64_t x_bs, const double* y, int64_t N,
                     int B, const double* u);
void sample_release(gpimhip_ctx* h);
int64_t sample_bytes(const gpimhip_ctx* h);
int fit_prologue(gpimhip_ctx* h, double lr, int T, double* adam_m, double* adam_v, size_t adam_bytes, int32_t* iter);
int plan_ensure(gpimhip_ctx* h, int nb);
int check_model(const gpimhip_model_t* m);
int launch_potrf(gpimhip_ctx* h, double* A, int64_t np, int64_t ld, int32_t* info);
int launch_trtri(gpimhip_ctx* h, double* A, double* Tm, int64_t np, int64_t ld);
int launch_potrf_inv(gpimhip_ctx* h, double* A, double* Tm, int64_t np, int64_t ld, int32_t* info, int rag);
int launch_lauum(gpimhip_ctx* h, const double* A, double* B, int64_t np, int64_t ld, int rag);
int upload_bc_table(gpimhip_ctx* h, double lr, int T);
int finish_and_check(gpimhip_ctx* h);
struct FitLoop { bool dense_gates, run_ahead; };
static const FitLoop FIT_LOOP_DENSE = {true, true}, FIT_LOOP_PLAIN = {false, false};
int run_fit_iterations(gpimhip_ctx* h, int T, FitLoop loop, const std::function<int()>& iteration);
void vfe_release(gpimhip_ctx* h);
void kron_release(gpimhip_ctx* h);
int launch_potrf_steps(gpimhip_ctx* h, double* A, int64_t np, int64_t ld, int32_t* info, double* Tm = nullptr, int rag = 0);
int launch_potrf_steps_f32(gpimhip_ctx* h, double* A, int64_t np, int64_t ld, int32_t* info);
void step_plan_release(gpimhip_ctx* h);
int step_plan_ensure(gpimhip_ctx* h, int nb);
int step_plan_ensure_inv(gpimhip_ctx* h, int nb);
int launch_panel_chain(gpimhip_ctx* h, double* A, int64_t ld, int p0, int p1, int nb, const TileDesc* tiles,
                       const PlanRange* colfill, int32_t* info);
int launch_dist_pack(gpimhip_ctx* h, const double* P, int64_t ldp, int64_t r0, int64_t np, int w, const double* dinv,
                     int nblk, double* buf, int64_t ldb);
int launch_colsumsq_acc(gpimhip_ctx* h, const double* W, int64_t ldw, int rows, int64_t m, double* q);
int launch_dist_trsv(gpimhip_ctx* h, const double* P, int64_t ld, const double* D, int nblk, int backward, const double* r0,
                     const double* r1, double* out);
int launch_dist_rows_acc(gpimhip_ctx* h, const double* A, int64_t ld, int64_t rows, int w, const double* x, double* acc);
#define GEMV_T_MULTI_RC 1024
static inline int gemv_t_multi_chunks(int64_t nrows) { return (int)((nrows + GEMV_T_MULTI_RC - 1) / GEMV_T_MULTI_RC); }
int multi_group_width(int ncols);
int launch_dist_trsv_multi(gpimhip_ctx* h, const double* P, int64_t ld, const double* D, int nblk, int backward, const double* r0,
                           int64_t r0_cs, const double* r1, int64_t r1_cs, int64_t r1_chs, int nch, int ncols, double* out,
                           int64_t out_cs);
int launch_dist_rows_acc_multi(gpimhip_ctx* h, const double* A, int64_t ld, int64_t rows, int w, const double* x, int64_t x_cs,
                               int ncols, double* acc, int64_t acc_cs);
int launch_gemv_t_multi(gpimhip_ctx* h, const double* A, int64_t ld, int64_t nrows, int w, const double* x, int64_t x_cs,
                        int ncols, double* part);
int launch_theta_raw(gpimhip_ctx* h, const gpimhip_model_t* m, const double* raw);
int launch_kmat(gpimhip_ctx* h, const gpimhip_model_t* m, const double* X, int64_t N, const double* Z,
                int64_t M, const ThetaDev* theta, double diag_add, int use_theta_diag, double* out,
                int64_t ld, int64_t rows_pad, int64_t cols_pad, int sym, int lower_only, int64_t x_bs,
                int64_t z_bs, int64_t out_bs);
int launch_pad_copy(gpimhip_ctx* h, const double* src, int64_t n, double* dst, int64_t np);
int launch_diag_inv_copy(gpimhip_ctx* h, double* A, int64_t ld, int nb);
int launch_pad_matrix_in(gpimhip_ctx* h, const double* src, int64_t n, int64_t ld, double* dst, int64_t np);
int launch_pad_matrix_out_lower(gpimhip_ctx* h, const double* src, int64_t np, double* dst, int64_t n, int64_t ld);
int launch_trmv_lower(gpimhip_ctx* h, const double* L, int64_t ld, int64_t np, const double* y, double* z);
int launch_gemv_t(gpimhip_ctx* h, const double* A, int64_t ld, int64_t nrows, int64_t ncols, const double* x,
                  double* out, int tri, int64_t a_bs, int64_t x_bs, int64_t o_bs);
int launch_grad_reduce(gpimhip_ctx* h, const gpimhip_model_t* m, const double* Kinv, int64_t ld,
                       const double* X, int64_t N, int nb, const double* alpha, int64_t x_bs);
int launch_kres(gpimhip_ctx* h, const gpimhip_model_t* m, const double* X, int64_t x_bs, int64_t N, double* scratch,
                int S, double* res);
int launch_axpy(gpimhip_ctx* h, double* x, const double* d, int64_t n);
int launch_gemv_t_tri(gpimhip_ctx* h, const double* A, int64_t ld, int64_t np, const double* x, double* part, double* out);
int launch_grad_reduce_fin(gpimhip_ctx* h, const gpimhip_model_t* m, const double* Kinv, int64_t ld, const double* X,
                           int64_t N, int nb, const double* alpha, int64_t x_bs, const double* alpha_part, double* u,
                           int do_adam, AdamStep st, double* loss_out, double* grad_out, double* hist_row, int32_t* iter,
                           const double* bc, int T, double* hist_base, double* loss_base, int carry_theta);
int launch_finalize(gpimhip_ctx* h, const gpimhip_model_t* m, int64_t N, int64_t np, double* u, int do_adam,
                    AdamStep st, double* loss_out, double* grad_out, double* hist_row, int32_t* iter,
                    const double* bc, int T, double* hist_base, double* loss_base, int carry_theta = 0);
int launch_predict_var(gpimhip_ctx* h, int64_t ldp, int nb, int64_t m0, int64_t mcount, double* var_out, int64_t M);
int launch_copy_slice(gpimhip_ctx* h, const double* src, double* dst, int64_t n, int64_t s_bs, int64_t d_bs);
int launch_acq(gpimhip_ctx* h, int kind, const double* mean, const double* sd, int64_t M, double p0, double p1,
               const double* mask, double* out);
int launch_nanmax(gpimhip_ctx* h, const double* x, int64_t n, double* out);
int launch_topk(gpimhip_ctx* h, const double* x, int64_t M, int k, int keep_nan, double* vals, int64_t* idx,
                int64_t* count);
int launch_grad_reduce_tiles(gpimhip_ctx* h, const gpimhip_model_t* m, const double* Kinv, int64_t ld, const double* X,
                             int64_t N, int64_t np, const double* alpha, const TileDesc* tiles, int ntile, double* part);
int launch_sum7(gpimhip_ctx* h, const double* part, int ntile, double* S);
int launch_kmat_refl(gpimhip_ctx* h, const gpimhip_model_t* m, const double* X, int64_t N, const double* Z, int64_t M,
                     const ThetaDev* theta, double* out, int64_t ld, int64_t rows_pad, int64_t cols_pad, int sym, int64_t x_bs,
                     int64_t z_bs, int64_t out_bs, double scale);
int launch_grad_reduce_refl(gpimhip_ctx* h, const gpimhip_model_t* m, const double* Kinv, int64_t ld, const double* X,
                            int64_t N, int nb, const double* alpha, int64_t x_bs);
int launch_finalize_coupled(gpimhip_ctx* h, const gpimhip_model_t* m, int64_t N, int64_t np, double* u, int do_adam,
                            AdamStep st, double* loss_out, double* grad_out, double* hist_row, int32_t* iter,
                            const double* bc, int T, double* hist_base, double* loss_base, const double* border_scal = nullptr);
int launch_coupled_sums(gpimhip_ctx* h, int64_t np, double* out11);
int launch_predict_coupled(gpimhip_ctx* h, int64_t ldp, int nb, int64_t m0, int64_t mcount, int64_t nvar, int64_t mean_bs,
                           double* mean_out, double* var_out, const double* radd = nullptr);
int launch_dist_finalize_dev(gpimhip_ctx* h, const gpimhip_model_t* m, int64_t N, const double* red, const double* quad,
                             double* u, int do_adam, AdamStep st, double* loss_out, double* grad_out, double* hist_row);
int launch_dist_finalize(gpimhip_ctx* h, const gpimhip_model_t* m, int64_t N, const double* S, double q2, double lg,
                         double* u, int do_adam, AdamStep st, double* loss_out, double* grad_out, double* hist_row);
int launch_add_diag_theta(gpimhip_ctx* h, double* out, int64_t ld, int64_t row0, int64_t n, int64_t npad);
int launch_theta(gpimhip_ctx* h, const gpimhip_model_t* m, const double* u);
int launch_topk_radix(gpimhip_ctx* h, const double* x, int64_t M, int k, int keep_nan, double* vals, int64_t* idx,
                      int64_t* count);
int launch_nanmax_two_stage(gpimhip_ctx* h, const double* x, int64_t n, double* out);
int launch_thin_batch(gpimhip_ctx* h, const double* vals, const int64_t* flat, int n, int d, const int64_t* shape,
                      double dscale, int max_out, int32_t* keep_out, int32_t* nkeep_out);
size_t sel_scratch_bytes();
int launch_fit_small(gpimhip_ctx* h, const gpimhip_model_t* m, const double* X, int64_t x_bs, const double* y,
                     int N, double* u, const double* lr_over_bc1, const double* bc2_sqrt, int T, double* hist,
                     double* loss, double* grad);
bool fused_predict_fits(int64_t np);
int launch_predict_fused(gpimhip_ctx* h, const gpimhip_model_t* m, const double* X, int64_t x_bs, int64_t N,
                         const double* Xs, int64_t M, double* mean_out, double* var_out, double* sd_out,
                         double* acq_out, int acq_kind, double p0, const double* p0_dev, double p1,
                         const double* mask);
int launch_acq_from_var(gpimhip_ctx* h, int kind, const double* mean, const double* var, int64_t M, double p0,
                        const double* p0_dev, double p1, const double* mask, double* sd_out, double* acq_out);


enum GemmEpi { EPI_STORE = 0, EPI_COLSUMSQ = 1 };
struct GemmArgs {
    const double* A; int64_t lda; int a_roff, a_coff;
    const double* B; int64_t ldb; int b_roff, b_coff;
    double* C; int64_t ldc; int c_roff, c_coff;
    double alpha, beta;
    const TileDesc* tiles; int ntiles;
    int cj_max;
    int cmap;
    int chunk;
    int inplace;
    int rag;
    int krev;
    int kfix0, kfix1;
    int rect_rows, rect_cols;
    double* colpart; int64_t ld_colpart;
    double* C2;
    int shape_div;
    int64_t sA, sB, sC, sColpart;
    int bshift;
};
int launch_gemm(gpimhip_ctx* h, bool a_km, bool b_km, int epi, const GemmArgs& g);
int launch_gemm_f32(gpimhip_ctx* h, bool a_km, bool b_km, int epi, const GemmArgs& g);
GemmArgs gemm_args(const double* A, int64_t lda, const double* B, int64_t ldb, double* C, int64_t ldc, double alpha, double beta,
                   const TileDesc* tiles, int n, int64_t rows);

enum GemmShape {
    GEMM_SHAPE_QUAD = GPIMHIP_GEMM_SHAPE_QUAD,
    GEMM_SHAPE_ROWHALF = GPIMHIP_GEMM_SHAPE_ROWHALF,
    GEMM_SHAPE_8W_LDS = GPIMHIP_GEMM_SHAPE_8W_LDS,
    GEMM_SHAPE_8W = GPIMHIP_GEMM_SHAPE_8W,
    GEMM_SHAPE_4W = GPIMHIP_GEMM_SHAPE_4W
};
static inline bool gemm_layout_ok(bool a_km, bool b_km, int epi) {
    if (epi == EPI_STORE) return !a_km || b_km;
    return epi == EPI_COLSUMSQ && !a_km && b_km;
}
int gemm_shape_f64(bool a_km, bool b_km, int epi, int64_t ntiles, int64_t batch, int shape_div, int inplace);
int gemm_shape_f32(bool a_km, bool b_km, int epi, int64_t ntiles, int64_t batch, int shape_div, int inplace);
int gemm_tile_pos_f32(int n, int chunk, int quads, int bx, int& quad);

template <int TSM, int TSN>
__host__ __device__ __forceinline__ int gemm_tile_pos(int n, int chunk, int bx, int& quad) {
    constexpr int QUADS = (128 / TSM) * (128 / TSN);
    const int b = bx / QUADS;
    quad = bx % QUADS;
    if (QUADS > 1) return b;
    if (chunk == 0) {
        const int q = n >> 3, r = n & 7, x = b & 7, yy = b >> 3;
        return (x < r ? x * (q + 1) : r * (q + 1) + (x - r) * q) + yy;
    }
    const int C = chunk, full = (n / (8 * C)) * (8 * C);
    if (b < full) {
        const int x = b & 7, y = b >> 3, round = y / C;
        return (round * 8 + ((round & 1) ? 7 - x : x)) * C + (y % C);
    }
    return b;
}
__host__ __device__ __forceinline__ void gemm_rect_tile(int rect_rows, int rect_cols, int p, int& ci, int& cj) {
    const int per = 8 * rect_cols, s = p / per, q = p - s * per, left = rect_rows - 8 * s, rows_here = left < 8 ? left : 8;
    ci = 8 * s + q % rows_here;
    cj = q / rows_here;
}
```

### gpim_amd/csrc/potf2_body.hpp

```cpp
#pragma once
#include "blocklds.hpp"

#ifdef POTF2_PROFILE
#define PROF_ARG , long long* __restrict__ prof
#define STAMP(i) do { if (threadIdx.x == 0) prof[i] = clock64(); } while (0)
#else
#define PROF_ARG
#define STAMP(i) do { } while (0)
#endif

#ifndef FI_BURST
#define FI_BURST 8
#endif
#ifdef FI_ROLE_VARIANTS
#include "../../tools/r6_role_variants.hpp"
#endif
#ifndef FI_LOOKAHEAD
#define FI_LOOKAHEAD 0
#endif
#define POTF2_SMEM_DOUBLES (LayTri::DOUBLES + NB + 32 * XS_LD + 4)
typedef LayTri PL;
template <typename R, bool LA = false>
__device__ __forceinline__ void potf2_body(double* __restrict__ smem, const int by, R* __restrict__ A, int64_t ld, int kblk,
                                           R* __restrict__ dinv_all, double* __restrict__ dinvB_all,
                                           double* __restrict__ logdet_out, int32_t* __restrict__ info, int nb PROF_ARG,
                                           int col_off = 0, bool inv_to_A = false) {
    double* D = smem;
    double* invd = D + PL::DOUBLES;
    double* Xs = invd + NB;
    double* red = Xs + 32 * XS_LD;
    int& s_bad = *reinterpret_cast<int*>(red + 2);
#ifdef FI_ROLE_VARIANTS
    int* fi_flags = reinterpret_cast<int*>(red + 2) + 1;
#endif
    A += (int64_t)by * nb * NB * ld;
    dinv_all += (int64_t)by * nb * NB * NB;
    logdet_out += (int64_t)by * nb;
    const int tid = threadIdx.x, lane = tid & 63, wave = __builtin_amdgcn_readfirstlane(tid >> 6);
    typedef R RV2 __attribute__((ext_vector_type(2)));
    R* Ablk = A + ((int64_t)kblk * NB) * ld + (int64_t)kblk * NB;
    if (tid == 0) s_bad = 0;
#ifdef FI_ROLE_VARIANTS
    if (tid < 3) fi_flags[tid] = 0;
#endif
    __syncthreads();
    STAMP(0);
    load_block_chol0(D, invd, &s_bad, Ablk, ld, tid, Xs);
    STAMP(1);
    auto lower_chunk = [&](int i, int e, int& r, int& c, bool factor_diag) {
        const int tj = e >> 7, rr = (e >> 3) & 15, c2 = (e & 7) * 2;
        r = i * 16 + rr;
        c = tj * 16 + c2;
        d2 v = (d2){0.0, 0.0};
        if (tj <= i) {
            if (factor_diag || !PL::XT) v = *reinterpret_cast<const d2*>(D + PL::tile(i, tj) + PL::in(rr, c2));
            else v = (d2){D[PL::tile(i, tj) + PL::in(c2, rr)], D[PL::tile(i, tj) + PL::in(c2 + 1, rr)]};
        }
        if (factor_diag && tj == i) {
            v[0] *= invd[c];
            v[1] *= invd[c + 1];
        }
        if (c > r) v[0] = 0.0;
        if (c + 1 > r) v[1] = 0.0;
        return v;
    };
    struct Sink {
        R* Ablk;
        int64_t ld;
        const double* D;
        const double* invd;
        __device__ __forceinline__ void tile(int t, int p, d4 acc, int lane) const {
            R* dst = Ablk + (int64_t)(16 * t + (lane & 15)) * ld + 16 * p + 2 * (lane >> 4);
            RV2 v;
            v[0] = (R)acc[0];
            v[1] = (R)acc[1];
            *reinterpret_cast<RV2*>(dst) = v;
            v[0] = (R)acc[2];
            v[1] = (R)acc[3];
            *reinterpret_cast<RV2*>(dst + 8) = v;
        }
        __device__ __forceinline__ void row(int i, int lane) const {
            const int c2 = (lane & 7) * 2;
            d2 w[2][2];
#pragma unroll
            for (int h = 0; h < 2; ++h) {
                const int rr = (lane >> 3) + 8 * h;
                w[0][h] = (i > 0) ? *reinterpret_cast<const d2*>(D + PL::tile(i, i - 1) + PL::in(rr, c2)) : (d2){0.0, 0.0};
                d2 v = *reinterpret_cast<const d2*>(D + PL::tile(i, i) + PL::in(rr, c2));
                v[0] = (c2 > rr) ? 0.0 : v[0] * invd[16 * i + c2];
                v[1] = (c2 + 1 > rr) ? 0.0 : v[1] * invd[16 * i + c2 + 1];
                w[1][h] = v;
            }
#pragma unroll
            for (int h = 0; h < 2; ++h) {
                R* dst = Ablk + (int64_t)(16 * i + (lane >> 3) + 8 * h) * ld + c2;
                RV2 v;
                if (i > 0) {
                    v[0] = (R)w[0][h][0];
                    v[1] = (R)w[0][h][1];
                    *reinterpret_cast<RV2*>(dst + 16 * (i - 1)) = v;
                }
                v[0] = (R)w[1][h][0];
                v[1] = (R)w[1][h][1];
                *reinterpret_cast<RV2*>(dst + 16 * i) = v;
                v[0] = (R)0.0;
                v[1] = (R)0.0;
                for (int tj = i + 1; tj < 8; ++tj) *reinterpret_cast<RV2*>(dst + 16 * tj) = v;
            }
        }
    };
    const Sink sink{Ablk, ld, D, invd};
#ifdef FI_ROLE_VARIANTS
    if (LA) lds_factor_inv_la<Sink>(D, invd, Xs, &s_bad, fi_flags, tid, sink);
    else
#endif
    lds_factor_inv<Sink, true, PL>(D, invd, Xs, 8, &s_bad, tid, sink);
    STAMP(2);
    if (wave < 2) {
        const double v = wave_sum(-log(invd[tid]));
        if (lane == 0) red[wave] = v;
    }
    __syncthreads();
    if (tid == 0) {
        logdet_out[kblk] = red[0] + red[1];
        if (s_bad != 0 && *info == 0) *info = col_off + kblk * NB + s_bad;
    }
    STAMP(3);
    STAMP(4);
    R* dinv = inv_to_A ? Ablk : dinv_all + (int64_t)kblk * NB * NB;
    const int64_t ldinv = inv_to_A ? ld : NB;
    for (int e = tid; e < NB * NB / 2; e += NTH) {
        int r, c;
        const d2 w = lower_chunk(e >> 10, e & 1023, r, c, false);
        RV2 v;
        v[0] = (R)w[0];
        v[1] = (R)w[1];
        *reinterpret_cast<RV2*>(dinv + r * ldinv + c) = v;
    }
    if (dinvB_all) {
        double* dB = dinvB_all + ((int64_t)by * nb + kblk) * (NB * NB);
        for (int e = tid; e < NB * NB / 2; e += NTH) {
            const int t = e >> 10, s2 = (e >> 6) & 15, l = e & 63;
            const int r = 16 * t + (l & 15), c = 8 * s2 + (l >> 4);
            const double* T = D + PL::tile(t, (s2 >> 1) <= t ? (s2 >> 1) : t);
            d2 v;
            v[0] = (c <= r) ? T[PL::XT ? PL::in(c & 15, r & 15) : PL::in(r & 15, c & 15)] : 0.0;
            v[1] = (c + 4 <= r) ? T[PL::XT ? PL::in((c + 4) & 15, r & 15) : PL::in(r & 15, (c + 4) & 15)] : 0.0;
            *reinterpret_cast<d2*>(dB + 2 * e) = v;
        }
    }
    STAMP(5);
}
```

### include/gpimhip.h

```cpp
#ifndef GPIMHIP_H
#define GPIMHIP_H

#include <stdint.h>

#ifdef __cplusplus
extern "C" {
#endif

#define GPIMHIP_OK            0
#define GPIMHIP_E_BADARG     -1
#define GPIMHIP_E_HIP        -2
#define GPIMHIP_E_NOT_PD     -3
#define GPIMHIP_E_NOMEM      -4

#define GPIMHIP_KERNEL_RBF       0
#define GPIMHIP_KERNEL_MATERN52  1
#define GPIMHIP_KERNEL_RQ        2

#define GPIMHIP_ACQ_CB   0
#define GPIMHIP_ACQ_EI   1
#define GPIMHIP_ACQ_POI  2

#define GPIMHIP_MAX_DIM  4
#define GPIMHIP_MAX_PARAMS 8

typedef struct gpimhip_ctx* gpimhip_handle;

typedef struct {
    int32_t kernel;
    int32_t dim;
    int32_t n_ls;
    int32_t reserved;
    double  amp_lo, amp_hi;
    double  ls_lo[GPIMHIP_MAX_DIM];
    double  ls_hi[GPIMHIP_MAX_DIM];
    double  jitter;
} gpimhip_model_t;

int  gpimhip_create(gpimhip_handle* out, int device, void* hip_stream);
int  gpimhip_destroy(gpimhip_handle h);
const char* gpimhip_last_error(void);
int  gpimhip_version(void);
int64_t gpimhip_workspace_bytes(gpimhip_handle h);


int gpimhip_kmat(gpimhip_handle h, const gpimhip_model_t* m,
                 const double* X, int64_t N, const double* Z, int64_t M,
                 const double* theta, double diag_add, double* out, int64_t ld);

int gpimhip_set_precision(gpimhip_handle h, int32_t bits);

int gpimhip_potrf(gpimhip_handle h, double* A, int64_t n, int64_t ld, int32_t* info);

int gpimhip_nll_grad(gpimhip_handle h, const gpimhip_model_t* m,
                     const double* X, const double* y, int64_t N,
                     const double* u, double* loss_out, double* grad_out);


int gpimhip_fit_exact(gpimhip_handle h, const gpimhip_model_t* m,
                      const double* X, const double* y, int64_t N,
                      double* u_inout, double lr, int32_t T,
                      double* hist_out, double* loss_out);

int gpimhip_predict_exact(gpimhip_handle h, const gpimhip_model_t* m,
                          const double* X, const double* y, int64_t N,
                          const double* u, const double* Xs, int64_t M,
                          double* mean_out, double* var_out);

int gpimhip_sample_exact(gpimhip_handle h, const gpimhip_model_t* m,
                         const double* X, const double* y, int64_t N, const double* u,
                         const double* Xs, int64_t M,
                         const double* Z, int32_t S,
                         int32_t noiseless, double jitter,
                         double* mean_out, double* var_out,
                         double* samples_out);

int gpimhip_sample_pathwise(gpimhip_handle h, const gpimhip_model_t* m,
                            const double* G, const int32_t* shape, int32_t mask, const double* twoc,
                            const int64_t* idx, const double* y, int64_t N, const double* u,
                            const double* Z, int32_t S,
                            int32_t noiseless, double jitter,
                            double* mean_out, double* samples_out);

int gpimhip_sample_blocks(gpimhip_handle h, const gpimhip_model_t* m,
                          const double* G, const int32_t* shape, int32_t mask, const double* twoc,
                          const double* y, const double* u,
                          const double* Z, int32_t S,
                          int32_t noiseless, double jitter,
                          double* mean_out, double* samples_out);

int gpimhip_sample_border(gpimhip_handle h, const gpimhip_model_t* m,
                          const double* X, int64_t x_stride, const double* y, int64_t N, int32_t B, const double* u,
                          const double* G, const int32_t* shape, int32_t mask, const double* twoc,
                          const int64_t* miss,
                          const double* Z, int32_t S,
                          int32_t noiseless, double jitter,
                          double* mean_out, double* samples_out);

int gpimhip_fit_exact_batched(gpimhip_handle h, const gpimhip_model_t* m,
                              const double* X, int64_t x_stride, const double* y, int64_t N, int32_t B,
                              double* u_inout, double lr, int32_t T,
                              double* hist_out, double* loss_out);
int gpimhip_predict_exact_batched(gpimhip_handle h, const gpimhip_model_t* m,
                                  const double* X, int64_t x_stride, const double* y, int64_t N, int32_t B,
                                  const double* u, const double* Xs, int64_t M,
                                  double* mean_out, double* var_out);

#define GPIMHIP_VGP_MAX_TASKS 16
typedef struct {
    int32_t tasks;
    int32_t rank;
    int32_t independent;
    int32_t ls_softplus;
} gpimhip_vgp_t;
int gpimhip_vgp_nll_grad(gpimhip_handle h, const gpimhip_model_t* m, const gpimhip_vgp_t* vg, const double* X,
                         const double* Y, int64_t N, const double* u, double* loss_out, double* grad_out);
int gpimhip_fit_vgp(gpimhip_handle h, const gpimhip_model_t* m, const gpimhip_vgp_t* vg, const double* X, const double* Y,
                    int64_t N, double* u_inout, double lr, int32_t T_iter, double* hist_out, double* loss_out);
int gpimhip_predict_vgp(gpimhip_handle h, const gpimhip_model_t* m, const gpimhip_vgp_t* vg, const double* X,
                        const double* Y, int64_t N, const double* u, const double* Xs, int64_t M, double* mean_out,
                        double* var_out);

int gpimhip_sample_vgp(gpimhip_handle h, const gpimhip_model_t* m, const gpimhip_vgp_t* vg,
                       const double* X, const double* Y, int64_t N, const double* u,
                       const double* Xs, int64_t M,
                       const double* Z, int32_t S,
                       int32_t noiseless, double jitter,
                       double* mean_out, double* var_out,
                       double* samples_out);
int gpimhip_sample_vgp_blocks(gpimhip_handle h, const gpimhip_model_t* m, const gpimhip_vgp_t* vg,
                              const double* G, const int32_t* shape, int32_t mask, const double* twoc,
                              const double* Y, const double* u,
                              const double* Z, int32_t S,
                              int32_t noiseless, double jitter,
                              double* mean_out, double* samples_out);

#define GPIMHIP_SM_MAX_MIXTURES 16
typedef struct {
    int32_t dim;
    int32_t mixtures;
    int32_t ard;
    int32_t reserved;
} gpimhip_sm_t;
int gpimhip_sm_kmat(gpimhip_handle h, const gpimhip_sm_t* sm, const double* X, int64_t N, const double* Z, int64_t M,
                    const double* u, double* out, int64_t ld);
int gpimhip_sm_nll_grad(gpimhip_handle h, const gpimhip_sm_t* sm, const double* X, const double* y, int64_t N,
                        const double* u, double* loss_out, double* grad_out);
int gpimhip_fit_sm(gpimhip_handle h, const gpimhip_sm_t* sm, const double* X, const double* y, int64_t N, double* u_inout,
                   double lr, int32_t T, double* hist_out, double* loss_out);
int gpimhip_predict_sm(gpimhip_handle h, const gpimhip_sm_t* sm, const double* X, const double* y, int64_t N,
                       const double* u, const double* Xs, int64_t M, double* mean_out, double* var_out);
int gpimhip_sample_sm(gpimhip_handle h, const gpimhip_sm_t* sm,
                      const double* X, const double* y, int64_t N, const double* u,
                      const double* Xs, int64_t M,
                      const double* Z, int32_t S,
                      int32_t noiseless, double jitter,
                      double* mean_out, double* var_out,
                      double* samples_out);
int gpimhip_sample_sm_pathwise(gpimhip_handle h, const gpimhip_sm_t* sm,
                               const double* G, const int32_t* shape, int32_t mask, const double* twoc,
                               const int64_t* idx, const double* y, int64_t N, const double* u,
                               const double* Z, int32_t S,
                               int32_t noiseless, double jitter,
                               double* mean_out, double* samples_out);
int gpimhip_sample_sm_blocks(gpimhip_handle h, const gpimhip_sm_t* sm,
                             const double* G, const int32_t* shape, int32_t mask, const double* twoc,
                             const double* y, const double* u,
                             const double* Z, int32_t S,
                             int32_t noiseless, double jitter,
                             double* mean_out, double* samples_out);
int gpimhip_sm_nll_grad_batched(gpimhip_handle h, const gpimhip_sm_t* sm, const double* X, const double* ys, const double* ones,
                                int64_t N, int32_t B, const double* u, double* loss_out, double* grad_out);
int gpimhip_fit_sm_batched(gpimhip_handle h, const gpimhip_sm_t* sm, const double* X, const double* ys, const double* ones,
                           int64_t N, int32_t B, double* u_inout, double lr, int32_t T, double* hist_out, double* loss_out);
int gpimhip_predict_sm_batched(gpimhip_handle h, const gpimhip_sm_t* sm, const double* X, const double* ys, const double* ones,
                               int64_t N, int32_t B, const double* u, const double* Xs, int64_t M, double* mean_out,
                               double* var_out);

int gpimhip_vfe_nll_grad(gpimhip_handle h, const gpimhip_model_t* m,
                         const double* X, const double* y, int64_t N, int64_t Mu,
                         const double* u, double* loss_out, double* grad_out);
int gpimhip_fit_vfe(gpimhip_handle h, const gpimhip_model_t* m,
                    const double* X, const double* y, int64_t N, int64_t Mu,
                    double* u_inout, double lr, int32_t T,
                    double* hist_theta, double* hist_xu, double* loss_out);
int gpimhip_predict_vfe(gpimhip_handle h, const gpimhip_model_t* m,
                        const double* X, const double* y, int64_t N, int64_t Mu,
                        const double* u, const double* Xs, int64_t M,
                        double* mean_out, double* var_out);
int gpimhip_fit_vfe_batched(gpimhip_handle h, const gpimhip_model_t* m,
                            const double* X, int64_t x_stride, const double* y, int64_t N, int64_t Mu, int32_t B,
                            double* u_inout, double lr, int32_t T,
                            double* hist_theta, double* hist_xu, double* loss_out);
int gpimhip_predict_vfe_batched(gpimhip_handle h, const gpimhip_model_t* m,
                                const double* X, int64_t x_stride, const double* y, int64_t N, int64_t Mu, int32_t B,
                                const double* u, const double* Xs, int64_t xs_stride, int64_t M,
                                double* mean_out, double* var_out);

int gpimhip_kron_nll_grad(gpimhip_handle h, const gpimhip_model_t* m, int32_t d, const int32_t* n,
                          const double* axes, const double* y, const double* u,
                          double* loss_out, double* grad_out);
int gpimhip_fit_kron(gpimhip_handle h, const gpimhip_model_t* m, int32_t d, const int32_t* n,
                     const double* axes, const double* y, double* u_inout, double lr, int32_t T,
                     double* hist_out, double* loss_out);
int gpimhip_predict_kron(gpimhip_handle h, const gpimhip_model_t* m, int32_t d, const int32_t* n,
                         const double* axes, const double* y, const double* u,
                         const int32_t* n_test, const double* axes_test,
                         double* mean_out, double* var_out);

int gpimhip_sample_kron(gpimhip_handle h, const gpimhip_model_t* m, int32_t d, const int32_t* n,
                        const double* axes, const double* y, const double* u,
                        const int32_t* n_test, const double* axes_test,
                        const int32_t* n_union, const double* axes_union,
                        const int32_t* idx_train, const int32_t* idx_test,
                        const double* z, int32_t S, int32_t noiseless, double jitter,
                        double* mean_out, double* out);

int gpimhip_pkron_nll_grad(gpimhip_handle h, const gpimhip_model_t* m, const double* Xs, int64_t Ns, int32_t p, int32_t dc,
                           const int32_t* n_c, const int32_t* perm, const double* axes_c, const double* Y, const double* u,
                           double* loss_out, double* grad_out);
int gpimhip_fit_pkron(gpimhip_handle h, const gpimhip_model_t* m, const double* Xs, int64_t Ns, int32_t p, int32_t dc,
                      const int32_t* n_c, const int32_t* perm, const double* axes_c, const double* Y, double* u_inout,
                      double lr, int32_t T, double* hist_out, double* loss_out);
int gpimhip_predict_pkron(gpimhip_handle h, const gpimhip_model_t* m, const double* Xs, int64_t Ns, int32_t p, int32_t dc,
                          const int32_t* n_c, const int32_t* perm, const double* axes_c, const double* Y, const double* u,
                          const double* Xs_test, int64_t Ms, const int32_t* n_test_c, const double* axes_test_c,
                          double* mean_out, double* var_out);

int gpimhip_sample_pkron(gpimhip_handle h, const gpimhip_model_t* m, const double* Xs, int64_t Ns, int32_t p, int32_t dc,
                         const int32_t* n_c, const int32_t* perm, const double* axes_c, const double* Y, const double* u,
                         const double* Xs_test, int64_t Ms, const int32_t* n_test_c, const double* axes_test_c,
                         const double* P, int64_t Us, const int32_t* irow_train, const int32_t* irow_test,
                         const int32_t* n_union, const double* axes_union, const int32_t* idx_train, const int32_t* idx_test,
                         const double* z, int32_t S, int32_t noiseless, double jitter, double* mean_out, double* samples_out);

int gpimhip_acq(gpimhip_handle h, int32_t kind, const double* mean, const double* sd,
                int64_t M, double p0, double p1, const double* mask, double* acq_out);

int gpimhip_acquire_exact(gpimhip_handle h, const gpimhip_model_t* m, const double* X, const double* y,
                          int64_t N, const double* u, const double* Xs, int64_t M, const double* Xobs,
                          int64_t Mobs, int32_t kind, double p0, double p1, const double* mask,
                          double* mean_out, double* sd_out, double* acq_out);

int gpimhip_nanmax(gpimhip_handle h, const double* x, int64_t n, double* out);

int gpimhip_topk(gpimhip_handle h, const double* acq, int64_t M, int32_t k, int32_t keep_nan,
                 double* vals_out, int64_t* idx_out, int64_t* count_out);

int gpimhip_dist_setup(gpimhip_handle h, int64_t n, int32_t world, int32_t rank);
int gpimhip_dist_begin(gpimhip_handle h, int64_t n);
int gpimhip_dist_panel_factor(gpimhip_handle h, double* Aloc, int64_t ldloc, int32_t loc_blk0,
                              int32_t glob_blk0, double* logdet_out, int32_t* info);
int gpimhip_dist_panel_pack(gpimhip_handle h, const double* Aloc, int64_t ldloc, int32_t loc_blk0,
                            int32_t glob_blk0, double* buf, int64_t ldbuf);
int gpimhip_dist_update(gpimhip_handle h, const double* buf, int64_t ldbuf, int32_t panel_glob_blk0,
                        double* Aloc, int64_t ldloc, int32_t panel_first, int32_t panel_last);
int gpimhip_dist_solve_update(gpimhip_handle h, const double* buf, int64_t ldbuf, int32_t panel_glob_blk0,
                              double* B, int64_t ldb, int64_t mpad, double* Wt, int64_t ldw, double* q,
                              int32_t col_tiles);
int gpimhip_dist_solve_update2(gpimhip_handle h, const double* wide, int64_t ldbuf, int32_t panel_glob_blk0, double* Bm,
                               int64_t ldb, int64_t mpad, double* Wt2, int64_t ldw, double* q, int32_t col_tiles,
                               int32_t second);

int gpimhip_dist_kmat_cols(gpimhip_handle h, const gpimhip_model_t* m, const double* X, int64_t N, const double* u,
                           int64_t col0, int64_t ncols_pad, double* out, int64_t ld);
int gpimhip_dist_vec_forward(gpimhip_handle h, const double* Aloc, int64_t ldloc, int32_t loc_blk0, int32_t glob_blk0,
                             const double* y_p, const double* t, double* piece, double* acc);
int gpimhip_dist_vec_backward(gpimhip_handle h, const double* Aloc, int64_t ldloc, int32_t loc_blk0, int32_t glob_blk0,
                              const double* z_p, const double* a, double* work, double* piece);
int gpimhip_matvec_t(gpimhip_handle h, const double* A, int64_t ld, int64_t nrows, int64_t ncols, const double* x,
                     double* out);
int gpimhip_dist_kinv_update(gpimhip_handle h, const double* xbuf, int64_t ldx, int32_t panel_glob_blk0,
                             const double* Xloc, int64_t ldloc, double* Kinv, int64_t ldk);
int gpimhip_dist_kinv_update_n(gpimhip_handle h, const double* xbuf, int64_t ldx, int32_t panel_glob_blk0, int32_t npanels,
                               const double* Xloc, int64_t ldloc, double* Kinv, int64_t ldk);
int gpimhip_dist_grad_sums(gpimhip_handle h, const gpimhip_model_t* m, const double* X, int64_t N, const double* u,
                           const double* Kinv, int64_t ldk, const double* alpha, double* S_out);
int gpimhip_dist_finalize(gpimhip_handle h, const gpimhip_model_t* m, int64_t N, double* u, const double* S,
                          double quad, double half_logdet, double lr, int32_t t, double* loss_out, double* grad_out,
                          double* hist_row);
int gpimhip_dist_finalize_dev(gpimhip_handle h, const gpimhip_model_t* m, int64_t N, double* u, const double* red,
                              const double* quad, double lr, int32_t t, double* loss_out, double* grad_out,
                              double* hist_row);

int gpimhip_set_reflection(gpimhip_handle h, int32_t mask, const double* twoc, const double* wts, int64_t n_total,
                           int64_t var_count);

int gpimhip_set_reflection_shard(gpimhip_handle h, int32_t pb_off, int32_t pb_stride, int32_t nblocks_total, int32_t raw);

int gpimhip_set_border(gpimhip_handle h, int32_t M, const int32_t* q, const double* coef);
int gpimhip_nll_grad_batched(gpimhip_handle h, const gpimhip_model_t* m, const double* X, int64_t x_stride, const double* y,
                             int64_t N, int32_t B, const double* u, double* loss_out, double* grad_out);
int gpimhip_refl_sums(gpimhip_handle h, const gpimhip_model_t* m, const double* X, const double* y, int64_t N, int32_t B,
                      const double* u, double* sums_out);

int gpimhip_thin_batch(gpimhip_handle h, const double* vals, const int64_t* flat_idx, int32_t n, int32_t d,
                       const int64_t* shape, double dscale, int32_t max_out, int32_t* keep_out,
                       int32_t* nkeep_out);

int gpimhip_step_plan_host(int32_t nb, int32_t with_inverse, int32_t* out, int64_t cap, int64_t* n_out);

int gpimhip_step_plan_host_f32(int32_t nb, int32_t with_inverse, int32_t* out, int64_t cap, int64_t* n_out,
                               int32_t* diag_out);

#define GPIMHIP_GEMM_SHAPE_QUAD 0
#define GPIMHIP_GEMM_SHAPE_ROWHALF 1
#define GPIMHIP_GEMM_SHAPE_8W_LDS 2
#define GPIMHIP_GEMM_SHAPE_8W 3
#define GPIMHIP_GEMM_SHAPE_4W 4
typedef struct {
    const void* A; int64_t lda; int32_t a_roff, a_coff;
    const void* B; int64_t ldb; int32_t b_roff, b_coff;
    void* C; int64_t ldc; int32_t c_roff, c_coff;
    double* colpart; int64_t ld_colpart;
    double alpha, beta;
    const int32_t* tiles; int32_t ntiles;
    int32_t a_km, b_km, epi;
    int32_t krev, chunk, kfix0, kfix1, rect_rows, rect_cols, cj_max, cmap, rag, inplace, bshift, shape_div;
    int64_t sA, sB, sC, sColpart;
    int32_t batch;
} gpimhip_gemm_test_t;
int gpimhip_gemm_tiles(gpimhip_handle h, const gpimhip_gemm_test_t* d);
int gpimhip_gemm_shape_host(int32_t fp32, int32_t a_km, int32_t b_km, int32_t epi, int64_t ntiles, int64_t batch,
                            int32_t shape_div, int32_t inplace);
int gpimhip_gemm_tile_pos_host(int32_t fp32, int32_t n, int32_t chunk, int32_t quads, int32_t bx0, int32_t count,
                               int32_t* p_out, int32_t* quad_out);
int gpimhip_gemm_rect_tile_host(int32_t rect_rows, int32_t rect_cols, int32_t p0, int32_t count, int32_t* ci_out,
                                int32_t* cj_out);

int gpimhip_kron_eigh(gpimhip_handle h, int32_t d, const int32_t* n, const double* axes, const double* ls, int32_t warm,
                      double* lam_out, double* Qt_out, int32_t* nprob_out, int32_t* plan_out, double* rot_out,
                      int32_t* cap_out);

int gpimhip_timing_enable(gpimhip_handle h, int enable);
int gpimhip_timing_read(gpimhip_handle h, int stage, double* total_ms, int64_t* count);

int gpimhip_fit_completed(gpimhip_handle h);

int gpimhip_shutdown(void);

int gpimhip_sync(gpimhip_handle h);

#ifdef __cplusplus
}
#endif
#endif
```

Measured before the change: 8744 grid-points/s.

## Factor two diagonal blocks per Cholesky step with paired panel solve and update

Adds a paired-step mode to the blocked f64 Cholesky (with inverse). On alternate columns a single hosted step kernel factors block j, bridges the j+1 panel and diagonal in-kernel, then factors block j+1. New panel_solve2 and diag_update2 kernels handle the two-column panel and trailing diagonal. The plan builder is extended so update and inverse tiles follow the paired schedule. The aim is to halve the number of serial potf2 launch steps on the critical path, at the cost of a longer serial chain inside each step and more complex planning.

```diff
diff --git a/gpim_amd/_lib.py b/gpim_amd/_lib.py
--- a/gpim_amd/_lib.py
+++ b/gpim_amd/_lib.py
@@ -198,6 +198,8 @@
                                         c_dp]),
     "gpimhip_step_plan_host": (ctypes.c_int, [ctypes.c_int32, ctypes.c_int32, ctypes.POINTER(ctypes.c_int32),
                                               ctypes.c_int64, ctypes.POINTER(ctypes.c_int64)]),
+    "gpimhip_step_plan_host_paired": (ctypes.c_int, [ctypes.c_int32, ctypes.POINTER(ctypes.c_int32), ctypes.c_int64,
+                                                     ctypes.POINTER(ctypes.c_int64), ctypes.POINTER(ctypes.c_int32)]),
     "gpimhip_step_plan_host_f32": (ctypes.c_int, [ctypes.c_int32, ctypes.c_int32, ctypes.POINTER(ctypes.c_int32),
                                                   ctypes.c_int64, ctypes.POINTER(ctypes.c_int64),
                                                   ctypes.POINTER(ctypes.c_int32)]),
diff --git a/gpim_amd/csrc/api.hip b/gpim_amd/csrc/api.hip
--- a/gpim_amd/csrc/api.hip
+++ b/gpim_amd/csrc/api.hip
@@ -69,6 +69,7 @@
     if (matrices) {
         rc = plan_ensure(h, (int)nb);
         if (rc == GPIMHIP_OK) rc = h->fp32 ? step_plan_ensure(h, (int)nb) : step_plan_ensure_inv(h, (int)nb);
+        if (rc == GPIMHIP_OK && !h->fp32) rc = step_plan_ensure_pair(h, (int)nb);
         if (rc != GPIMHIP_OK) { ws_release_matrix(h); return rc; }
     }
     return GPIMHIP_OK;
diff --git a/gpim_amd/csrc/cholstep.hip b/gpim_amd/csrc/cholstep.hip
--- a/gpim_amd/csrc/cholstep.hip
+++ b/gpim_amd/csrc/cholstep.hip
@@ -22,11 +22,11 @@
     GemmArgs g;
 };
 
-template <int FTM, int FTN, bool ALONE, bool RAG = false>
+template <int FTM, int FTN, bool ALONE, bool RAG = false, bool PAIR = false>
 __global__ __launch_bounds__(NTH, ALONE ? 2 : 4) void chol_step_kernel(StepArgs a) {
     constexpr int SM0 = POTF2_SMEM_DOUBLES > gemm_smem_doubles<FTM, FTN, 2>() ? POTF2_SMEM_DOUBLES : gemm_smem_doubles<FTM, FTN, 2>();
     static_assert(SM0 * 8 <= 80 * 1024, "two workgroups per CU");
-    constexpr int SM = ALONE ? 84 * 128 : SM0;
+    constexpr int SM = ALONE ? 84 * 128 : SM0 + (PAIR ? 2 : 0);
     __shared__ __attribute__((aligned(16))) double smem[SM];
     const int b = a.swap ? blockIdx.y : blockIdx.x;
     const int by = a.swap ? blockIdx.x : blockIdx.y;
@@ -57,8 +57,21 @@
     }
     if (b != 0 || !a.potf2 || by >= a.pb_cnt) return;
     if (!ALONE) __builtin_amdgcn_s_setprio(3);
+    int* wave_counter = reinterpret_cast<int*>(smem + POTF2_SMEM_DOUBLES);
+    if (PAIR && threadIdx.x == 0) *wave_counter = 0;
     potf2_body<double, ALONE && FI_LOOKAHEAD>(smem, by + a.pb_off, a.A, a.ld, a.kblk, a.dinv_all, a.dinvB_all, a.logdet, a.info, a.nb,
                                               a.col_off, a.Tm != nullptr);
+    if (PAIR) {
+        const volatile __attribute__((address_space(4))) StepArgs* ka =
+            (const volatile __attribute__((address_space(4))) StepArgs*)__builtin_amdgcn_kernarg_segment_ptr();
+        const int tid2 = pair_tid(wave_counter);
+        double* A2 = ka->A;
+        const int64_t ld2 = ka->ld;
+        const int k2 = ka->kblk, nb2 = ka->nb, pb2 = (ka->swap ? blockIdx.x : blockIdx.y) + ka->pb_off;
+        pair_bridge(smem, pb2, A2, ld2, k2, nb2, ka->Pcopy, tid2);
+        potf2_body<double, ALONE && FI_LOOKAHEAD>(smem, pb2, A2, ld2, k2 + 1, ka->dinv_all, ka->dinvB_all, ka->logdet, ka->info, nb2,
+                                                  ka->col_off, ka->Tm != nullptr, tid2);
+    }
 }
 
 template <int WPE>
@@ -269,6 +282,146 @@
     for (int rg = 0; rg < 4; ++rg) C[(int64_t)(4 * rg) * ld] = cv[rg] - (acc0[rg] + acc1[rg]);
 }
 
+__global__ __launch_bounds__(256, 2) void panel_solve2_kernel(double* __restrict__ A, int64_t ld, int kblk, int nb,
+                                                             const double* __restrict__ dinvB_all,
+                                                             const double* __restrict__ LB_all, int b_off) {
+    constexpr int LDS_LD = 130, ROWS = 32, MTS = ROWS / 16;
+    __shared__ __attribute__((aligned(16))) double S[2 * ROWS * LDS_LD];
+    const int tid = threadIdx.x, lane = tid & 63, wave = tid >> 6;
+    const int by = blockIdx.y + b_off;
+    A += (int64_t)by * nb * NB * ld;
+    const d2* DB = reinterpret_cast<const d2*>(dinvB_all + ((int64_t)by * nb + kblk) * (NB * NB));
+    const d2* LB = reinterpret_cast<const d2*>(LB_all + (int64_t)by * (NB * NB));
+    double* P = A + ((int64_t)(kblk + 2) * NB + (int64_t)blockIdx.x * ROWS) * ld + (int64_t)kblk * NB;
+    double* S1 = S + ROWS * LDS_LD;
+#pragma unroll
+    for (int i = 0; i < ROWS / 4; ++i) {
+        const int row = wave * (ROWS / 4) + i;
+        __builtin_amdgcn_global_load_lds((const __attribute__((address_space(1))) void*)(P + (int64_t)row * ld + lane * 2),
+                                         (__attribute__((address_space(3))) void*)(S + row * LDS_LD), 16, 0, 0);
+        __builtin_amdgcn_global_load_lds((const __attribute__((address_space(1))) void*)(P + (int64_t)row * ld + NB + lane * 2),
+                                         (__attribute__((address_space(3))) void*)(S1 + row * LDS_LD), 16, 0, 0);
+    }
+    const int t0 = wave, t1 = 7 - wave, n0 = 2 * t0 + 2;
+    const d4 zero = (d4){0.0, 0.0, 0.0, 0.0};
+    const double* Sa = S + (lane & 15) * LDS_LD + (lane >> 4);
+#pragma unroll
+    for (int c = 0; c < 2; ++c) {
+        d2 bf[18];
+#pragma unroll
+        for (int q = 0; q < 18; ++q) {
+            const int t = q < n0 ? t0 : t1, s2 = q < n0 ? q : q - n0;
+            bf[q] = DB[c * (NB * NB / 2) + (t * 16 + s2) * 64 + lane];
+        }
+        asm volatile("s_waitcnt vmcnt(0)" ::: "memory");
+        __syncthreads();
+        d4 acc[2][MTS];
+#pragma unroll
+        for (int x = 0; x < 2; ++x)
+#pragma unroll
+            for (int mt = 0; mt < MTS; ++mt) acc[x][mt] = zero;
+#pragma unroll
+        for (int q = 0; q < 18; ++q) {
+            const bool first = q < n0;
+            const int s2 = first ? q : q - n0;
+#pragma unroll
+            for (int e = 0; e < 2; ++e) {
+                const int s = 2 * s2 + e;
+#pragma unroll
+                for (int mt = 0; mt < MTS; ++mt) {
+                    const double av = Sa[c * ROWS * LDS_LD + mt * 16 * LDS_LD + 4 * s];
+                    if (first) acc[0][mt] = __builtin_amdgcn_mfma_f64_16x16x4f64(av, bf[q][e], acc[0][mt], 0, 0, 0);
+                    else acc[1][mt] = __builtin_amdgcn_mfma_f64_16x16x4f64(av, bf[q][e], acc[1][mt], 0, 0, 0);
+                }
+            }
+        }
+#pragma unroll
+        for (int x = 0; x < 2; ++x) {
+            const int t = x == 0 ? t0 : t1;
+#pragma unroll
+            for (int mt = 0; mt < MTS; ++mt)
+#pragma unroll
+                for (int rg = 0; rg < 4; ++rg)
+                    P[(int64_t)(mt * 16 + (lane >> 4) + 4 * rg) * ld + c * NB + t * 16 + (lane & 15)] = acc[x][mt][rg];
+        }
+        if (c == 1) break;
+        __syncthreads();
+#pragma unroll
+        for (int x = 0; x < 2; ++x) {
+            const int t = x == 0 ? t0 : t1;
+#pragma unroll
+            for (int mt = 0; mt < MTS; ++mt)
+#pragma unroll
+                for (int rg = 0; rg < 4; ++rg)
+                    S[(mt * 16 + (lane >> 4) + 4 * rg) * LDS_LD + t * 16 + (lane & 15)] = acc[x][mt][rg];
+        }
+        __syncthreads();
+#pragma unroll
+        for (int x = 0; x < 2; ++x) {
+            const int t = x == 0 ? t0 : t1;
+            d2 lb[16];
+#pragma unroll
+            for (int s2 = 0; s2 < 16; ++s2) lb[s2] = LB[(t * 16 + s2) * 64 + lane];
+            d4 u[MTS];
+#pragma unroll
+            for (int mt = 0; mt < MTS; ++mt) u[mt] = zero;
+#pragma unroll
+            for (int s2 = 0; s2 < 16; ++s2)
+#pragma unroll
+                for (int e = 0; e < 2; ++e)
+#pragma unroll
+                    for (int mt = 0; mt < MTS; ++mt)
+                        u[mt] = __builtin_amdgcn_mfma_f64_16x16x4f64(Sa[mt * 16 * LDS_LD + 4 * (2 * s2 + e)], lb[s2][e], u[mt], 0, 0, 0);
+#pragma unroll
+            for (int mt = 0; mt < MTS; ++mt)
+#pragma unroll
+                for (int rg = 0; rg < 4; ++rg) S1[(mt * 16 + (lane >> 4) + 4 * rg) * LDS_LD + t * 16 + (lane & 15)] -= u[mt][rg];
+        }
+    }
+}
+
+__global__ __launch_bounds__(256, 2) void diag_update2_kernel(double* __restrict__ A, int64_t ld, int kblk, int nb, int b_off) {
+    constexpr int LDS_LD = 130;
+    __shared__ __attribute__((aligned(16))) double S[64 * LDS_LD];
+    const int tid = threadIdx.x, lane = tid & 63, wave = tid >> 6;
+    A += (int64_t)(blockIdx.y + b_off) * nb * NB * ld;
+    const int q = blockIdx.x;
+    int a = 0;
+    while ((a + 1) * (a + 2) / 2 <= q) ++a;
+    const int b = q - a * (a + 1) / 2;
+    const int64_t r0 = (int64_t)(kblk + 2) * NB;
+    const double* Pa = A + (r0 + a * 32) * ld + (int64_t)kblk * NB;
+    const double* Pb = A + (r0 + b * 32) * ld + (int64_t)kblk * NB;
+    const int wm = wave >> 1, wn = wave & 1;
+    double* C = A + (r0 + a * 32 + wm * 16 + (lane >> 4)) * ld + r0 + b * 32 + wn * 16 + (lane & 15);
+    double cv[4];
+#pragma unroll
+    for (int rg = 0; rg < 4; ++rg) cv[rg] = C[(int64_t)(4 * rg) * ld];
+    d4 acc0 = (d4){0.0, 0.0, 0.0, 0.0}, acc1 = acc0;
+    const double* Sa = S + (wm * 16 + (lane & 15)) * LDS_LD + (lane >> 4);
+    const double* Sb = S + (32 + wn * 16 + (lane & 15)) * LDS_LD + (lane >> 4);
+    for (int h = 0; h < 2; ++h) {
+        if (h) __syncthreads();
+#pragma unroll
+        for (int i = 0; i < 8; ++i) {
+            const int row = wave * 8 + i;
+            __builtin_amdgcn_global_load_lds((const __attribute__((address_space(1))) void*)(Pa + (int64_t)row * ld + h * NB + lane * 2),
+                                             (__attribute__((address_space(3))) void*)(S + row * LDS_LD), 16, 0, 0);
+            __builtin_amdgcn_global_load_lds((const __attribute__((address_space(1))) void*)(Pb + (int64_t)row * ld + h * NB + lane * 2),
+                                             (__attribute__((address_space(3))) void*)(S + (32 + row) * LDS_LD), 16, 0, 0);
+        }
+        asm volatile("s_waitcnt vmcnt(0)" ::: "memory");
+        __syncthreads();
+#pragma unroll
+        for (int s = 0; s < 32; s += 2) {
+            acc0 = __builtin_amdgcn_mfma_f64_16x16x4f64(Sa[4 * s], Sb[4 * s], acc0, 0, 0, 0);
+            acc1 = __builtin_amdgcn_mfma_f64_16x16x4f64(Sa[4 * s + 4], Sb[4 * s + 4], acc1, 0, 0, 0);
+        }
+    }
+#pragma unroll
+    for (int rg = 0; rg < 4; ++rg) C[(int64_t)(4 * rg) * ld] = cv[rg] - (acc0[rg] + acc1[rg]);
+}
+
 static void lower_patches(std::vector<TileDesc>& out, int lo, int hi, int kb0, int kb1) {
     for (int ig = lo / 8; ig <= (hi - 1) / 8; ++ig)
         for (int jg = lo / 8; jg <= ig; ++jg)
@@ -309,7 +462,7 @@
 #define HOST_SLOTS 512
 static double wg_cost(int depth, int q) { return q == 4 ? 0.14 * depth + 0.24 : (q == 2 ? 0.34 * depth + 0.3 : depth + 0.5); }
 
-static void plan_updates(int nb, std::vector<std::vector<TileDesc>>& fill) {
+static void plan_updates(int nb, std::vector<std::vector<TileDesc>>& fill, std::vector<uint8_t>* lead = nullptr) {
 #ifndef STEP_W_CHAIN
 #define STEP_W_CHAIN 3
 #endif
@@ -319,15 +472,27 @@
     const int W = (nb >= STEP_W_CHAIN_MIN && nb < 64) ? STEP_W_CHAIN : STEP_W, S = HOST_SLOTS;
     const int npanel = (nb + W - 1) / W;
     auto by_depth = [](const TileDesc& a, const TileDesc& b) { return (a.kb1 - a.kb0) > (b.kb1 - b.kb0); };
-    auto col_update = [&](std::vector<TileDesc>& tl, int p0, int j) {
+    auto col_update = [&](std::vector<TileDesc>& tl, int p0, int j, bool after_pair = false) {
         const int kb0 = std::max(0, p0 - W);
         if (j > kb0)
-            for (int i = j + 1; i < nb; ++i) tl.push_back({i, j, kb0, j});
-        if (j + 1 < nb) {
+            for (int i = j + 1 + (after_pair ? 1 : 0); i < nb; ++i) tl.push_back({i, j, kb0, j});
+        if (j + 1 < nb && !after_pair) {
             const int kd = std::max(0, ((j + 1) / W) * W - W);
             if (j > kd) tl.push_back({j + 1, j + 1, kd, j});
         }
     };
+    auto col_update_pair = [&](std::vector<TileDesc>& tl, int p0, int j) {
+        const int kb0 = std::max(0, p0 - W);
+        if (j > kb0)
+            for (int c = j; c <= j + 1; ++c)
+                for (int i = j + 2; i < nb; ++i) tl.push_back({i, c, kb0, j});
+        for (int c = j + 2; c <= j + 3; ++c) {
+            const int kd = std::max(0, (c / W) * W - W);
+            if (j > kd)
+                for (int i = c; i <= j + 3; ++i) tl.push_back({i, c, kd, j});
+        }
+    };
+    if (lead) lead->assign(nb, 0);
     if (nb < 64) {
         for (int p = 0; p < npanel; ++p) {
             const int p0 = p * W, p1 = std::min(p0 + W, nb), ncol = p1 - p0;
@@ -372,10 +537,13 @@
                 if (due(t)) { ++n_due; due_cost += HostSim::cost(t); }
         }
         size_t rtaken = 0, otaken = 0;
+        const bool paired = lead && bulk_regime;
         for (int j = p0; j < p1; ++j) {
-            const int left = p1 - j;
+            if (paired && ((j - p0) & 1)) { (*lead)[j] = 2; continue; }
+            const int left = paired ? (p1 - j + 1) / 2 : p1 - j;
             std::vector<TileDesc>& tl = fill[j];
-            col_update(tl, p0, j);
+            if (paired) { (*lead)[j] = 1; col_update_pair(tl, p0, j); }
+            else col_update(tl, p0, j, lead && j == p0 && j >= 2 && (*lead)[j - 2] == 1);
             const size_t nreq = (req.size() - rtaken + left - 1) / left;
             for (size_t q = 0; q < nreq; ++q) tl.push_back(req[rtaken++]);
             if (!bulk_regime) {
@@ -383,7 +551,7 @@
                 for (size_t q = 0; q < nopt; ++q) tl.push_back(opt[otaken++]);
             } else {
                 HostSim sim(S);
-                sim.add(1.0);
+                sim.add(paired ? 2.5 : 1.0);
                 std::stable_sort(tl.begin(), tl.end(), by_depth);
                 double base = 0.0;
                 for (auto& t : tl) { sim.add(HostSim::cost(t)); base += HostSim::cost(t); }
@@ -449,7 +617,7 @@
 #endif
 static bool pair_rule(size_t ntiles, int64_t kblocks) { return 4 * ntiles >= PAIR_MIN_QUADS && 10 * kblocks >= PAIR_MIN_DEPTH10 * (int64_t)ntiles; }
 static bool plan_inverse(int nb, std::vector<std::vector<TileDesc>>& fill, std::vector<std::vector<TileDesc>>& post,
-                         std::vector<uint8_t>& pair) {
+                         std::vector<uint8_t>& pair, const std::vector<uint8_t>* lead = nullptr) {
     std::vector<TriNodeS> nodes;
     tri_nodes(0, nb, nodes);
     std::vector<int> order(nodes.size());
@@ -463,6 +631,8 @@
     const double CHAIN = PLAN_CHAIN;
     for (int L = 0; open_nodes > 0; ++L) {
         const bool hosted = L < nb;
+        if (hosted && lead && (*lead)[L] == 2) continue;
+        const bool leader = hosted && lead && (*lead)[L] == 1;
         if (!hosted) post.emplace_back();
         std::vector<TileDesc>& out = hosted ? fill[L] : post.back();
         int64_t upd = 0;
@@ -477,7 +647,7 @@
 #ifndef PLAN_PAIR_CHAIN
 #define PLAN_PAIR_CHAIN 0.3
 #endif
-        const double slow = two ? PLAN_PAIR_SLOW : 1.0, chain = two ? CHAIN + PLAN_PAIR_CHAIN : CHAIN;
+        const double slow = two ? PLAN_PAIR_SLOW : 1.0, chain = leader ? 2 * CHAIN + 0.5 : (two ? CHAIN + PLAN_PAIR_CHAIN : CHAIN);
         HostSim sim(q == 1 || two ? HOST_SLOTS : HOST_SLOTS / 2);
         double target = 1e30;
         if (hosted) {
@@ -560,7 +730,9 @@
     }
 }
 
-static int step_plan_build(gpimhip_ctx* h, int nb, StepPlan& P, bool with_inverse) {
+static bool pair_steps_apply(int nb) { return nb >= 64 + STEP_W; }
+
+static int step_plan_build(gpimhip_ctx* h, int nb, StepPlan& P, bool with_inverse, bool paired = false) {
     const bool fp32 = h->fp32 != 0;
     if (P.nb == nb && P.fp32 == (int)fp32) return GPIMHIP_OK;
     if (P.d_tiles) { (void)hipFree(P.d_tiles); P.d_tiles = nullptr; }
@@ -568,14 +740,15 @@
     const int npanel = (nb + W - 1) / W;
     std::vector<std::vector<TileDesc>> fill(nb), post, rest(npanel);
     std::vector<int> ndiag32;
-    if (!fp32) plan_updates(nb, fill);
+    if (!fp32) plan_updates(nb, fill, paired ? &P.lead : nullptr);
     else plan_updates_f32(nb, fill, rest, ndiag32);
+    if (!paired) P.lead.assign(nb, 0);
     P.n_update.assign(nb, 0);
     for (int j = 0; j < nb; ++j)
         for (auto& t : fill[j]) P.n_update[j] += t.kb1 - t.kb0;
     P.pair.assign(nb, 0);
     if (with_inverse) {
-        if (!plan_inverse(nb, fill, post, P.pair)) {
+        if (!plan_inverse(nb, fill, post, P.pair, paired ? &P.lead : nullptr)) {
             gpim_set_error("step plan: the inverse's tile operations did not all find a launch (nb = " + std::to_string(nb) + ")");
             return GPIMHIP_E_BADARG;
         }
@@ -640,6 +813,30 @@
     return GPIMHIP_OK;
 }
 
+extern "C" int gpimhip_step_plan_host_paired(int32_t nb, int32_t* out, int64_t cap, int64_t* n_out, int32_t* pair_out) {
+    if (nb < 1 || nb > 4096 || !n_out) return GPIMHIP_E_BADARG;
+    std::vector<std::vector<TileDesc>> fill(nb), post;
+    std::vector<uint8_t> lead(nb, 0), pair(nb, 0);
+    const bool paired = pair_steps_apply(nb);
+    plan_updates(nb, fill, paired ? &lead : nullptr);
+    if (!plan_inverse(nb, fill, post, pair, paired ? &lead : nullptr)) return GPIMHIP_E_BADARG;
+    int64_t n = 0;
+    for (int j = 0; j < nb; ++j) n = emit_plan_records(j, fill[j], out, cap, n);
+    for (size_t q = 0; q < post.size(); ++q) n = emit_plan_records(nb + (int)q, post[q], out, cap, n);
+    for (int j = 0; j < nb; ++j) {
+        if (lead[j] != 1) continue;
+        std::vector<TileDesc> fd2;
+        for (int i = j + 2; i < nb; ++i) fd2.push_back({i, j + 1, j, (j + 1) | (5 << 16)});
+        for (int c = j + 2; c <= j + 3; ++c)
+            for (int i = c; i <= j + 3; ++i) fd2.push_back({i, c, j, (j + 2) | (5 << 16)});
+        n = emit_plan_records(j, fd2, out, cap, n);
+    }
+    if (pair_out)
+        for (int j = 0; j < nb; ++j) pair_out[j] = lead[j];
+    *n_out = n;
+    return GPIMHIP_OK;
+}
+
 extern "C" int gpimhip_step_plan_host_f32(int32_t nb, int32_t with_inverse, int32_t* out, int64_t cap, int64_t* n_out,
                                           int32_t* diag_out) {
     if (nb < 1 || nb > 4096 || !n_out) return GPIMHIP_E_BADARG;
@@ -660,9 +857,13 @@
 
 int step_plan_ensure(gpimhip_ctx* h, int nb) { return step_plan_build(h, nb, h->splan, false); }
 int step_plan_ensure_inv(gpimhip_ctx* h, int nb) { return step_plan_build(h, nb, h->splan_inv, true); }
+int step_plan_ensure_pair(gpimhip_ctx* h, int nb) {
+    if (h->fp32 || !pair_steps_apply(nb) || getenv("GPIMHIP_NO_PAIR_STEPS") != nullptr) return GPIMHIP_OK;
+    return step_plan_build(h, nb, h->splan_pair, true, true);
+}
 
 void step_plan_release(gpimhip_ctx* h) {
-    for (StepPlan* P : {&h->splan, &h->splan_inv}) {
+    for (StepPlan* P : {&h->splan, &h->splan_inv, &h->splan_pair}) {
         if (P->d_tiles) (void)hipFree(P->d_tiles);
         P->d_tiles = nullptr;
         P->nb = 0;
@@ -678,7 +879,8 @@
     return g;
 }
 
-static int launch_step(gpimhip_ctx* h, StepArgs& a, bool potf2, int n, int q, const int* split = nullptr, bool two_per_cu = false) {
+static int launch_step(gpimhip_ctx* h, StepArgs& a, bool potf2, int n, int q, const int* split = nullptr, bool two_per_cu = false,
+                       bool lead = false) {
     const int B = h->nbatch;
     a.potf2 = potf2 ? 1 : 0;
     if (!potf2 && n == 0) return GPIMHIP_OK;
@@ -693,7 +895,23 @@
         if (grid.x == 0) return GPIMHIP_OK;
         if (grid.y > 65535) { gpim_set_error("step launch: tile list too long for a split batch"); return GPIMHIP_E_BADARG; }
     }
-    if (a.g.rag && n) {
+    if (lead) {
+        if (!potf2 || split) { gpim_set_error("step launch: a pair leader is a single-batch launch with the factorisation role"); return GPIMHIP_E_BADARG; }
+        const bool rag = a.g.rag && n;
+        if (q == 4 && alone) {
+            if (rag) hipLaunchKernelGGL((chol_step_kernel<64, 64, true, true, true>), grid, dim3(NTH), 0, h->stream, a);
+            else hipLaunchKernelGGL((chol_step_kernel<64, 64, true, false, true>), grid, dim3(NTH), 0, h->stream, a);
+        } else if (q == 4) {
+            if (rag) hipLaunchKernelGGL((chol_step_kernel<64, 64, false, true, true>), grid, dim3(NTH), 0, h->stream, a);
+            else hipLaunchKernelGGL((chol_step_kernel<64, 64, false, false, true>), grid, dim3(NTH), 0, h->stream, a);
+        } else if (q == 2) {
+            if (rag) hipLaunchKernelGGL((chol_step_kernel<128, 64, false, true, true>), grid, dim3(NTH), 0, h->stream, a);
+            else hipLaunchKernelGGL((chol_step_kernel<128, 64, false, false, true>), grid, dim3(NTH), 0, h->stream, a);
+        } else {
+            if (rag) hipLaunchKernelGGL((chol_step_kernel<128, 128, false, true, true>), grid, dim3(NTH), 0, h->stream, a);
+            else hipLaunchKernelGGL((chol_step_kernel<128, 128, false, false, true>), grid, dim3(NTH), 0, h->stream, a);
+        }
+    } else if (a.g.rag && n) {
         if (q == 4 && alone) hipLaunchKernelGGL((chol_step_kernel<64, 64, true, true>), grid, dim3(NTH), 0, h->stream, a);
         else if (q == 4) hipLaunchKernelGGL((chol_step_kernel<64, 64, false, true>), grid, dim3(NTH), 0, h->stream, a);
         else if (q == 2) hipLaunchKernelGGL((chol_step_kernel<128, 64, false, true>), grid, dim3(NTH), 0, h->stream, a);
@@ -734,14 +952,24 @@
     return GPIMHIP_OK;
 }
 
+static int launch_solve_diag2(gpimhip_ctx* h, double* A, int64_t ld, int j, int nb, int b_off, int cnt) {
+    hipLaunchKernelGGL(panel_solve2_kernel, dim3(4 * (nb - j - 2), cnt), dim3(256), 0, h->stream, A, ld, j, nb,
+                       (const double*)h->dinvB, (const double*)h->pcopy, b_off);
+    HIP_TRY(hipGetLastError());
+    hipLaunchKernelGGL(diag_update2_kernel, dim3(36, cnt), dim3(256), 0, h->stream, A, ld, j, nb, b_off);
+    HIP_TRY(hipGetLastError());
+    return GPIMHIP_OK;
+}
+
 int launch_potrf_steps(gpimhip_ctx* h, double* A, int64_t np, int64_t ld, int32_t* info, double* Tm, int rag) {
     if (h->fp32) return launch_potrf_steps_f32(h, A, np, ld, info);
     const int nb = (int)(np / NB);
+    const int B = h->nbatch;
+    const int host_max_batch = 4;
+    const bool paired = Tm && B <= host_max_batch && h->pcopy && h->splan_pair.d_tiles && h->splan_pair.nb == nb && h->splan_pair.fp32 == 0;
     if (Tm) GP_TRY(step_plan_ensure_inv(h, nb));
     else GP_TRY(step_plan_ensure(h, nb));
-    const StepPlan& P = Tm ? h->splan_inv : h->splan;
-    const int B = h->nbatch;
-    const int host_max_batch = 4;
+    const StepPlan& P = paired ? h->splan_pair : (Tm ? h->splan_inv : h->splan);
     StepArgs a;
     a.A = A; a.ld = ld; a.nb = nb; a.Tm = Tm;
     a.dinv_all = h->dinv; a.dinvB_all = h->dinvB; a.logdet = h->logdet_part; a.info = info;
@@ -778,11 +1006,16 @@
             }
         } else {
             for (int j = 0; j < nb; ++j) {
+                if (P.lead[j] == 2) continue;
                 a.kblk = j;
                 int q;
                 const int nf = hosted_list(j, B, q);
-                GP_TRY(launch_step(h, a, true, nf, q, nullptr, P.pair[j] != 0));
-                GP_TRY(launch_solve_diag(h, A, ld, j, nb, P.diag[j].n, 0, B, fused(j)));
+                GP_TRY(launch_step(h, a, true, nf, q, nullptr, P.pair[j] != 0, P.lead[j] == 1));
+                if (P.lead[j] == 1) {
+                    GP_TRY(launch_solve_diag2(h, A, ld, j, nb, 0, B));
+                } else {
+                    GP_TRY(launch_solve_diag(h, A, ld, j, nb, P.diag[j].n, 0, B, fused(j)));
+                }
             }
         }
     }
diff --git a/gpim_amd/csrc/common.hpp b/gpim_amd/csrc/common.hpp
--- a/gpim_amd/csrc/common.hpp
+++ b/gpim_amd/csrc/common.hpp
@@ -97,6 +97,7 @@
     std::vector<int32_t> n_all;
     std::vector<uint8_t> pair;
     std::vector<uint8_t> copy;
+    std::vector<uint8_t> lead;
 };
 
 struct DistPlan {
@@ -161,6 +162,7 @@
     int64_t bytes = 0;
     LinalgPlan plan;
     StepPlan splan, splan_inv;
+    StepPlan splan_pair;
     DistPlan dplan;
     bool timing = false;
     std::vector<std::pair<hipEvent_t, hipEvent_t>> ev[7];
@@ -287,6 +289,7 @@
 void step_plan_release(gpimhip_ctx* h);
 int step_plan_ensure(gpimhip_ctx* h, int nb);
 int step_plan_ensure_inv(gpimhip_ctx* h, int nb);
+int step_plan_ensure_pair(gpimhip_ctx* h, int nb);
 int launch_panel_chain(gpimhip_ctx* h, double* A, int64_t ld, int p0, int p1, int nb, const TileDesc* tiles,
                        const PlanRange* colfill, int32_t* info);
 int launch_dist_pack(gpimhip_ctx* h, const double* P, int64_t ldp, int64_t r0, int64_t np, int w, const double* dinv,
diff --git a/gpim_amd/csrc/potf2_body.hpp b/gpim_amd/csrc/potf2_body.hpp
--- a/gpim_amd/csrc/potf2_body.hpp
+++ b/gpim_amd/csrc/potf2_body.hpp
@@ -24,7 +24,7 @@
 __device__ __forceinline__ void potf2_body(double* __restrict__ smem, const int by, R* __restrict__ A, int64_t ld, int kblk,
                                            R* __restrict__ dinv_all, double* __restrict__ dinvB_all,
                                            double* __restrict__ logdet_out, int32_t* __restrict__ info, int nb PROF_ARG,
-                                           int col_off = 0, bool inv_to_A = false) {
+                                           int col_off = 0, bool inv_to_A = false, int tid_in = -1) {
     double* D = smem;
     double* invd = D + PL::DOUBLES;
     double* Xs = invd + NB;
@@ -36,7 +36,7 @@
     A += (int64_t)by * nb * NB * ld;
     dinv_all += (int64_t)by * nb * NB * NB;
     logdet_out += (int64_t)by * nb;
-    const int tid = threadIdx.x, lane = tid & 63, wave = __builtin_amdgcn_readfirstlane(tid >> 6);
+    const int tid = tid_in < 0 ? (int)threadIdx.x : tid_in, lane = tid & 63, wave = __builtin_amdgcn_readfirstlane(tid >> 6);
     typedef R RV2 __attribute__((ext_vector_type(2)));
     R* Ablk = A + ((int64_t)kblk * NB) * ld + (int64_t)kblk * NB;
     if (tid == 0) s_bad = 0;
@@ -151,3 +151,84 @@
     }
     STAMP(5);
 }
+
+__device__ __forceinline__ int pair_tid(int* counter) {
+    const int lane = __builtin_amdgcn_mbcnt_hi(~0u, __builtin_amdgcn_mbcnt_lo(~0u, 0u));
+    int w = 0;
+    if (lane == 0) w = atomicAdd(counter, 1);
+    w = __builtin_amdgcn_readfirstlane(w);
+    int tid = w * 64 + lane;
+    asm volatile("" : "+v"(tid));
+    return tid;
+}
+
+__device__ __forceinline__ void pair_bridge(const double* smem, const int by, double* A, int64_t ld, int kblk, int nb, double* LB,
+                                            const int tid) {
+    const double* D = smem;
+    A += (int64_t)by * nb * NB * ld;
+    LB += (int64_t)by * (NB * NB);
+    const int lane = tid & 63, wave = __builtin_amdgcn_readfirstlane(tid >> 6);
+    const int n = lane & 15, kq = lane >> 4;
+    double* P = A + ((int64_t)(kblk + 1) * NB) * ld + (int64_t)kblk * NB;
+    double* C = P + NB;
+    __syncthreads();
+    {
+        double af[32];
+        const double* Pa = P + (int64_t)(16 * wave + n) * ld + kq;
+#pragma unroll
+        for (int s = 0; s < 32; ++s) af[s] = Pa[4 * s];
+#pragma unroll 1
+        for (int t = 0; t < 8; ++t) {
+            d4 acc = (d4){0.0, 0.0, 0.0, 0.0};
+            const double* Dt = D + PL::tile(t, 0);
+#pragma unroll
+            for (int sc = 0; sc < 8; ++sc) {
+                if (sc <= t) {
+#pragma unroll
+                    for (int e = 0; e < 4; ++e) {
+                        const int kk = 4 * e + kq;
+                        double b = Dt[sc * 256 + (PL::XT ? PL::in(kk, n) : PL::in(n, kk))];
+                        if (sc == t && kk > n) b = 0.0;
+                        acc = __builtin_amdgcn_mfma_f64_16x16x4f64(af[4 * sc + e], b, acc, 0, 0, 0);
+                    }
+                }
+            }
+#pragma unroll
+            for (int rg = 0; rg < 4; ++rg) {
+                const int rr = kq + 4 * rg, c = 16 * t + n;
+                P[(int64_t)(16 * wave + rr) * ld + c] = acc[rg];
+                LB[(((wave * 16 + (c >> 3)) * 64 + (((c & 3) << 4) | rr)) << 1) + ((c >> 2) & 1)] = acc[rg];
+            }
+        }
+    }
+    asm volatile("s_waitcnt vmcnt(0)" ::: "memory");
+    __syncthreads();
+    __builtin_amdgcn_fence(__ATOMIC_ACQUIRE, "agent");
+    const d2* LB2 = reinterpret_cast<const d2*>(LB);
+    for (int q = wave; q < 36; q += 8) {
+        int mt = 0;
+        while ((mt + 1) * (mt + 2) / 2 <= q) ++mt;
+        const int nt = q - mt * (mt + 1) / 2;
+        d4 acc0 = (d4){0.0, 0.0, 0.0, 0.0}, acc1 = acc0;
+#pragma unroll 1
+        for (int h = 0; h < 2; ++h) {
+            d2 fa[8], fb[8];
+#pragma unroll
+            for (int s2 = 0; s2 < 8; ++s2) {
+                fa[s2] = LB2[(mt * 16 + 8 * h + s2) * 64 + lane];
+                fb[s2] = LB2[(nt * 16 + 8 * h + s2) * 64 + lane];
+            }
+#pragma unroll
+            for (int s2 = 0; s2 < 8; ++s2) {
+                acc0 = __builtin_amdgcn_mfma_f64_16x16x4f64(fa[s2][0], fb[s2][0], acc0, 0, 0, 0);
+                acc1 = __builtin_amdgcn_mfma_f64_16x16x4f64(fa[s2][1], fb[s2][1], acc1, 0, 0, 0);
+            }
+        }
+        double* Cp = C + (int64_t)(16 * mt + kq) * ld + 16 * nt + n;
+#pragma unroll
+        for (int rg = 0; rg < 4; ++rg) Cp[(int64_t)(4 * rg) * ld] = Cp[(int64_t)(4 * rg) * ld] - (acc0[rg] + acc1[rg]);
+    }
+    asm volatile("s_waitcnt vmcnt(0)" ::: "memory");
+    __syncthreads();
+    __builtin_amdgcn_fence(__ATOMIC_ACQUIRE, "agent");
+}
diff --git a/include/gpimhip.h b/include/gpimhip.h
--- a/include/gpimhip.h
+++ b/include/gpimhip.h
@@ -300,6 +300,8 @@
 
 int gpimhip_step_plan_host(int32_t nb, int32_t with_inverse, int32_t* out, int64_t cap, int64_t* n_out);
 
+int gpimhip_step_plan_host_paired(int32_t nb, int32_t* out, int64_t cap, int64_t* n_out, int32_t* pair_out);
+
 int gpimhip_step_plan_host_f32(int32_t nb, int32_t with_inverse, int32_t* out, int64_t cap, int64_t* n_out,
                                int32_t* diag_out);
 
```

New measurement: 8841 grid-points/s (median of 6 runs). 1.1% higher.
